# Frankie2030/DataMining_RecBLR

Hardware: AMD Instinct MI355X
Metric: sequences/sec fwd+bwd at B=2048 L=200 d=128; 1/2/4/8-GPU scaling (higher is better)
Workload: dtype f32 I/O, f16x3 split GEMM products

## Files before the change

datamining_recblr_amd/_lib.py:

```python
from __future__ import annotations

import ctypes
import os
import re
import threading

_HERE = os.path.dirname(os.path.abspath(__file__))
LIB_PATH = os.environ.get("RECBLR_LIB") or os.path.join(_HERE, "lib", "libdmrecblr.so")
HEADER_PATH = os.path.join(os.path.dirname(_HERE), "include", "recblr_hip.h")


class RecBLRNativeError(RuntimeError):
    """The HIP extension is missing, failed to load, or a kernel call failed."""


_BY_VALUE = {"int": ctypes.c_int, "int64_t": ctypes.c_int64, "uint64_t": ctypes.c_uint64,
             "float": ctypes.c_float, "double": ctypes.c_double}
_NOT_DECLARATIONS = re.compile(
    r'/\*.*?\*/|//[^\n]*|^[ \t]*#[^\n]*|\btypedef\b(?:[^;{]|\{[^}]*\})*;|extern\s+"C"\s*\{|^\s*\}\s*$',
    re.S | re.M)


def parse_header(text: str) -> dict:
    out = {}
    for decl in _NOT_DECLARATIONS.sub(" ", text).split(";"):
        decl = " ".join(decl.split())
        if not decl:
            continue
        m = re.fullmatch(r"([\w\s*]+?)\s*\b(\w+)\s*\(([^()]*)\)", decl)
        if m is None:
            raise RecBLRNativeError(f"header: not a plain function declaration: {decl!r}")
        ret, name, params = m.groups()
        if re.fullmatch(r"const\s+char\s*\*", ret):
            restype = ctypes.c_char_p
        elif ret in _BY_VALUE:
            restype = _BY_VALUE[ret]
        else:
            raise RecBLRNativeError(f"header: {name}: unsupported return type {ret!r}")
        argtypes = []
        for param in ([] if params.strip() == "void" else params.split(",")):
            words = param.split()
            by_value = " ".join(words[:-1] if len(words) > 1 else words)
            if "*" in param:
                argtypes.append(ctypes.c_void_p)
            elif by_value in _BY_VALUE:
                argtypes.append(_BY_VALUE[by_value])
            else:
                raise RecBLRNativeError(f"header: {name}: unsupported parameter {param.strip()!r}")
        out[name] = (restype, argtypes)
    return out


def _read(path: str) -> str:
    with open(path) as f:
        return f.read()


def _define(text: str, name: str) -> int:
    m = re.search(rf"^[ \t]*#[ \t]*define[ \t]+{name}[ \t]+\(?(-?\d+)\)?[ \t]*$", text, re.M)
    if m is None:
        raise RecBLRNativeError(f"header: no integer #define {name}")
    return int(m.group(1))


_header = _read(HEADER_PATH)
RB_EINVAL = _define(_header, "RB_EINVAL")
RB_TILE = _define(_header, "RB_TILE")
ABI_VERSION = _define(_header, "RB_ABI_VERSION")

SIGNATURES = parse_header(_header)
EXP_SIGNATURES = parse_header(_read(os.path.join(_HERE, "experimental", "recblr_exp.h")))
PROBE_SIGNATURES = parse_header(_read(os.path.join(_HERE, "probes", "recblr_probe.h")))
SESSION_SIGNATURES = parse_header(_read(os.path.join(_HERE, "session", "recblr_session.h")))

_lock = threading.Lock()
_loaded = {}


def _load(path, signatures, missing, version=None, mismatch=None, cache=True,
          hint="") -> ctypes.CDLL:
    with _lock:
        if cache and path in _loaded:
            return _loaded[path]
        if not os.path.exists(path):
            raise RecBLRNativeError(f"{missing}: {path} is missing. Run "
                                    f"`python -m datamining_recblr_amd.build`{hint}.")
        try:
            lib = ctypes.CDLL(path)
        except OSError as exc:
            raise RecBLRNativeError(f"failed to load {path}: {exc}") from exc
        for name, (res, args) in signatures.items():
            fn = getattr(lib, name)
            fn.restype = res
            fn.argtypes = args
        if version is not None and getattr(lib, version)() != ABI_VERSION:
            raise RecBLRNativeError(mismatch.format(getattr(lib, version)(), ABI_VERSION))
        if cache:
            _loaded[path] = lib
        return lib


def load(path: str | None = None) -> ctypes.CDLL:
    return _load(path or LIB_PATH, SIGNATURES, "HIP extension not built", "rb_version",
                 "ABI mismatch: library {} vs binding {}; rebuild", cache=path is None,
                 hint=" (hipcc --offload-arch=gfx950)")


def load_probe() -> ctypes.CDLL:
    return _load(os.path.join(os.path.dirname(LIB_PATH), "libdmrecblr_probe.so"),
                 PROBE_SIGNATURES, "probe library not built")


def load_exp() -> ctypes.CDLL:
    return _load(os.path.join(os.path.dirname(LIB_PATH), "libdmrecblr_exp.so"), EXP_SIGNATURES,
                 "experimental library not built", "rb_exp_version",
                 "experimental library ABI {} vs {}; rebuild")


def load_session() -> ctypes.CDLL:
    return _load(os.path.join(os.path.dirname(LIB_PATH), "libdmrecblr_session.so"),
                 SESSION_SIGNATURES, "session library not built", "rb_session_version",
                 "session library ABI {} vs {}; rebuild")


_fns = {}
_failure_hooks = []


def on_failure(hook) -> None:
    _failure_hooks.append(hook)


def _check(rc: int, name: str, lib: ctypes.CDLL, last_error: str, hooks: bool = True) -> None:
    if rc == 0:
        return
    kind = str(rc)
    if hooks:
        for hook in _failure_hooks:
            hook()
        kind = "invalid argument" if rc == RB_EINVAL else f"hipError {rc}"
    msg = getattr(lib, last_error)()
    raise RecBLRNativeError(f"{name} failed ({kind}): {msg.decode() if msg else ''}")


def call(name: str, *args) -> None:
    fn = _fns.get(name)
    if fn is None:
        fn = _fns[name] = getattr(load(), name)
    rc = fn(*args)
    if rc != 0:
        _check(rc, name, load(), "rb_last_error_string")


def call_probe(name: str, *args) -> None:
    lib = load_probe()
    _check(getattr(lib, name)(*args), name, lib, "rb_probe_last_error_string", hooks=False)
# ... 13 lines not shown
```

datamining_recblr_amd/blocks.py:

```python
from __future__ import annotations

import os

import torch
import torch.nn.functional as F

from . import kernels
from ._lib import RecBLRNativeError
from .linear import (_timed, fire_hooks, has_hooks, linear, mm_nn, mm_nn_dact, mm_nn_dact_ok, mm_nt,
                     mm_nt_act, mm_nt_act_ok, mm_nt_ln, mm_nt_ln_ok, rmax_buffer, wgrad)

__all__ = ["draw_seed", "ResidualGrad", "add_dropout_layer_norm", "embed_dropout_layer_norm",
           "linear_add_dropout_layer_norm", "silu_dropout", "feed_forward", "set_defer_residual",
           "defer_residual"]


_GOLDEN = 0x9E3779B97F4A7C15


def _rank() -> int:
    dist = torch.distributed
    return dist.get_rank() if dist.is_available() and dist.is_initialized() else 0


def draw_seed() -> int:
    s = int(torch.randint(0, 2 ** 62, (1,), dtype=torch.int64).item())
    r = _rank()
    if r:
        s = (s + r * _GOLDEN) % (2 ** 62)
    return s


def _drop(dropout: torch.nn.Dropout, training: bool):
    p = float(dropout.p) if training else 0.0
    return p, (draw_seed() if p > 0.0 else 0)


def _require_gpu(t):
    if t.device.type != "cuda":
        raise RecBLRNativeError(
            "the RecBLR blocks run on the MI355X HIP path only (ROCm GPU tensors)")


class ResidualGrad:
    __slots__ = ("ds", "rows", "taken")

    def __init__(self, rows=None):
        self.ds = None
        self.rows = rows
        self.taken = False


_defer_residual = [os.environ.get("RECBLR_DEFER_RESIDUAL", "1") != "0"]


def set_defer_residual(on: bool) -> None:
    _defer_residual[0] = bool(on)


def defer_residual() -> bool:
    return _defer_residual[0]


# ... 87 lines not shown
        flat = idx.reshape(-1).contiguous()
        plan = None
        if ctx.needs_input_grad[0]:
            plan = kernels.embedding_plan(flat, table.shape[0], table.shape[1])
        y, s, mean, rstd = kernels.add_ln_fwd(table, None, gamma, beta, eps, mask=mask,
                                              seed=seed, p=p, idx=flat, save=save)
        ctx.seed, ctx.p = seed, p
        ctx.padding_idx, ctx.num_rows = padding_idx, table.shape[0]
        ctx.plan = plan
        ctx.addend = _take(addend)
        ctx.save_for_backward(s, mean, rstd, gamma, mask, flat)
        return y.view(*idx.shape, table.shape[1])

    @staticmethod
    def backward(ctx, dy):
        s, mean, rstd, gamma, mask, flat = ctx.saved_tensors
        _, da, dg, db, _ = kernels.add_ln_bwd(dy, s, gamma, mean, rstd, mask=mask,
                                              seed=ctx.seed, p=ctx.p, want_ds=False,
                                              want_da=True, dy2=_pop(ctx.addend))
        dtable = None
        if ctx.needs_input_grad[0]:
            dtable = kernels.embedding_bwd(flat, da, ctx.num_rows, ctx.padding_idx,
                                           plan=ctx.plan)
            ctx.plan = None
        return dtable, None, dg, db, None, None, None, None, None, None


class _SiluDropout(torch.autograd.Function):
    @staticmethod
    def forward(ctx, a, mask, seed, p):
        a = a.contiguous()
        ctx.seed, ctx.p = seed, p
        ctx.save_for_backward(a, mask)
        return kernels.silu_dropout_fwd(a, mask=mask, seed=seed, p=p)

    @staticmethod
    def backward(ctx, du):
        a, mask = ctx.saved_tensors
        da, _ = kernels.silu_dropout_bwd(a, du, mask=mask, seed=ctx.seed, p=ctx.p)
        return da, None, None, None


class _FeedForward(torch.autograd.Function):

    @staticmethod
    def forward(ctx, x, w1, b1, w2, b2, gamma, beta, seed1, seed2, p, eps, in_addend=None,
                out_addend=None, observe=None):
        d = x.shape[-1]
        x2 = x.reshape(-1, d)
        M, inner = x2.shape[0], w1.shape[0]
        f = 2 * M * d * inner
        want = ctx.needs_input_grad[1] or ctx.needs_input_grad[3]
        r_x = rmax_buffer(x2, inner, d) if want else None
        if mm_nt_act_ok(x2, w1):
            (a1, u), a1_bias = _timed("gemm", f, mm_nt_act, x2, w1, b1, seed1, p, rmax=r_x), None
        else:
            a1 = _timed("gemm", f, mm_nt, x2, w1, rmax=r_x)
            u = kernels.silu_dropout_fwd(a1, seed=seed1, p=p, bias=b1)
            a1_bias = b1
        r_u = rmax_buffer(u, d, inner) if want else None
        save = any(ctx.needs_input_grad)
        x2c = x2.contiguous()
        if observe is None and mm_nt_ln_ok(u, w2):
            y, s, mean, rstd = _timed("gemm", f, mm_nt_ln, u, w2, b2, x2c, gamma, beta, eps,
                                      seed2, p, rmax=r_u)
        else:
            a2 = _timed("gemm", f, mm_nt, u, w2, b2, rmax=r_u)
            if observe is not None:
                pre = a1 if a1_bias is None else a1 + a1_bias
                observe(x2.view(x.shape), pre.view(*x.shape[:-1], inner),
                        u.view(*x.shape[:-1], inner), a2.view(x.shape))
            y, s, mean, rstd = kernels.add_ln_fwd(a2, x2c, gamma, beta, eps, seed=seed2, p=p,
                                                  save=save)
        ctx.r_x, ctx.r_u = r_x, r_u
        ctx.seed1, ctx.seed2, ctx.p = seed1, seed2, p
        ctx.a1_has_bias = a1_bias is None
        ctx.in_addend = in_addend if in_addend is not None and in_addend.taken else None
        ctx.out_addend = _take(out_addend)
        ctx.save_for_backward(x2, a1, u, s, mean, rstd, w1, b1, w2, gamma)
        return y.view(x.shape)

    @staticmethod
    def backward(ctx, dy):
        x2, a1, u, s, mean, rstd, w1, b1, w2, gamma = ctx.saved_tensors
        M, d = x2.shape
        f = 2 * M * d * w1.shape[0]
        ds, da2, dgamma, dbeta, db2 = kernels.add_ln_bwd(
            dy, s, gamma, mean, rstd, seed=ctx.seed2, p=ctx.p, want_ds=True, want_da=True,
            want_dbias=True, dy2=_pop(ctx.out_addend))
        r_da2 = rmax_buffer(da2, w2.shape[1], d) if ctx.r_u is not None else None
        if ctx.a1_has_bias and mm_nn_dact_ok(da2, w2):
            da1, db1 = _timed("gemm", f, mm_nn_dact, da2, w2, a1, ctx.seed1, ctx.p, rmax=r_da2)
            dw2 = _timed("gemm", f, wgrad, da2, u, ymax=r_da2, xmax=ctx.r_u)
        else:
            du = _timed("gemm", f, mm_nn, da2, w2, rmax=r_da2)
            dw2 = _timed("gemm", f, wgrad, da2, u, ymax=r_da2, xmax=ctx.r_u)
            da1, db1 = kernels.silu_dropout_bwd(a1, du, seed=ctx.seed1, p=ctx.p, want_dbias=True,
                                                bias=None if ctx.a1_has_bias else b1)
        r_da1 = rmax_buffer(da1, d, w1.shape[0]) if ctx.r_x is not None else None
        dx = _timed("gemm", f, mm_nn, da1, w1, rmax=r_da1)
        if ctx.in_addend is not None:
            ctx.in_addend.ds = ds
        else:
            dx.add_(ds)
        dw1 = _timed("gemm", f, wgrad, da1, x2, ymax=r_da1, xmax=ctx.r_x)
        return (dx.view(dy.shape), dw1, db1, dw2, db2, dgamma, dbeta, None, None, None, None,
                None, None, None)


def add_dropout_layer_norm(a, residual, dropout: torch.nn.Dropout, ln: torch.nn.LayerNorm,
                           training: bool, slot: ResidualGrad | None = None,
                           addend: ResidualGrad | None = None):
    _require_gpu(a)
    if a.shape[-1] not in kernels.ROW_SIZES:
        return ln(dropout(a) + residual)
    p, seed = _drop(dropout, training)
    return _AddDropoutLN.apply(a, residual, ln.weight, ln.bias, None, seed, p, ln.eps, slot,
                               addend)


def linear_add_dropout_layer_norm(x, proj: torch.nn.Linear, residual, dropout: torch.nn.Dropout,
                                  ln: torch.nn.LayerNorm, training: bool,
                                  slot: ResidualGrad | None = None,
                                  addend: ResidualGrad | None = None):
    _require_gpu(x)
    x2 = x.reshape(-1, x.shape[-1])
    if proj.bias is None and ln.weight.shape[0] == proj.weight.shape[0] and mm_nt_ln_ok(x2, proj.weight):
        p, seed = _drop(dropout, training)
        return _LinearAddDropoutLN.apply(x, proj.weight, residual, ln.weight, ln.bias, seed, p,
                                         ln.eps, slot, addend)
    return add_dropout_layer_norm(proj(x), residual, dropout, ln, training, slot, addend)


def embed_dropout_layer_norm(idx, emb: torch.nn.Embedding, dropout: torch.nn.Dropout,
                             ln: torch.nn.LayerNorm, training: bool,
                             addend: ResidualGrad | None = None):
    _require_gpu(emb.weight)
    if emb.weight.shape[1] not in kernels.ROW_SIZES:
        return ln(dropout(emb(idx)))
    p, seed = _drop(dropout, training)
    return _EmbedDropoutLN.apply(emb.weight, idx, ln.weight, ln.bias, None, seed, p, ln.eps,
                                 emb.padding_idx, addend)


def silu_dropout(a, dropout: torch.nn.Dropout, training: bool):
    _require_gpu(a)
    if a.shape[-1] not in kernels.ROW_SIZES:
        return dropout(F.silu(a))
    p, seed = _drop(dropout, training)
    return _SiluDropout.apply(a, None, seed, p)

# ... 20 lines not shown
```

datamining_recblr_amd/build.py:

```python
from __future__ import annotations

import glob
import os
import shutil
import subprocess
import sys

_HERE = os.path.dirname(os.path.abspath(__file__))
ROOT = os.path.dirname(_HERE)
SOURCES = sorted(glob.glob(os.path.join(_HERE, "csrc", "*.hip")))
HEADERS = sorted(glob.glob(os.path.join(_HERE, "csrc", "*.h"))) + [
    os.path.join(ROOT, "include", "recblr_hip.h")]
OUT = os.path.join(_HERE, "lib", "libdmrecblr.so")
PROBE_SOURCES = sorted(glob.glob(os.path.join(_HERE, "probes", "*.hip")))
PROBE_HEADERS = HEADERS + sorted(glob.glob(os.path.join(_HERE, "probes", "*.h")))
PROBE_OUT = os.path.join(_HERE, "lib", "libdmrecblr_probe.so")
EXP_SOURCES = sorted(glob.glob(os.path.join(_HERE, "experimental", "*.hip")))
EXP_HEADERS = HEADERS + sorted(glob.glob(os.path.join(_HERE, "experimental", "*.h")))
EXP_OUT = os.path.join(_HERE, "lib", "libdmrecblr_exp.so")
SESSION_SOURCES = sorted(glob.glob(os.path.join(_HERE, "session", "*.hip")))
SESSION_HEADERS = HEADERS + sorted(glob.glob(os.path.join(_HERE, "session", "*.h")))
SESSION_OUT = os.path.join(_HERE, "lib", "libdmrecblr_session.so")
ARCH = os.environ.get("PYTORCH_ROCM_ARCH", "gfx950")

FLAGS = ["-O3", "-std=c++20", "-shared", "-fPIC", f"--offload-arch={ARCH}",
         "-ffp-contract=off", "-Wall", "-Wno-unused-function"]


def hipcc() -> str:
    for cand in (os.environ.get("HIPCC"), "/opt/rocm/bin/hipcc", shutil.which("hipcc")):
        if cand and os.path.exists(cand):
            return cand
    raise RuntimeError("hipcc not found (expected /opt/rocm/bin/hipcc)")


def _stale(out, deps) -> bool:
    if not os.path.exists(out):
        return True
    t = os.path.getmtime(out)
    return any(os.path.getmtime(s) > t for s in deps)


def _compile(out, sources, extra, verbose, jobs):
    os.makedirs(os.path.dirname(out), exist_ok=True)
    tmp = out + ".tmp"
    cmd = [hipcc(), *FLAGS, *extra, "-I", os.path.join(ROOT, "include"), "-o", tmp, *sources]
    if jobs > 1:
        cmd.insert(1, f"-parallel-jobs={jobs}")
    if verbose:
        print(" ".join(cmd), flush=True)
    subprocess.run(cmd, check=True)
    os.replace(tmp, out)


def build(force: bool = False, verbose: bool = False, jobs: int = 4) -> str:
    if force or _stale(OUT, SOURCES + HEADERS):
        _compile(OUT, SOURCES, [], verbose, jobs)
    if PROBE_SOURCES and (force or _stale(PROBE_OUT, PROBE_SOURCES + PROBE_HEADERS)):
        _compile(PROBE_OUT, PROBE_SOURCES, ["-fvisibility=hidden"], verbose, jobs)
    if EXP_SOURCES and (force or _stale(EXP_OUT, EXP_SOURCES + EXP_HEADERS)):
        _compile(EXP_OUT, EXP_SOURCES, ["-fvisibility=hidden"], verbose, jobs)
    if SESSION_SOURCES and (force or _stale(SESSION_OUT, SESSION_SOURCES + SESSION_HEADERS)):
        _compile(SESSION_OUT, SESSION_SOURCES, ["-fvisibility=hidden"], verbose, jobs)
    return OUT

# ... 4 lines not shown
```

datamining_recblr_amd/csrc/capi.hip:

```cpp
#include "common.h"

#include <atomic>

namespace rb {

namespace {
thread_local std::string g_last_error;
}

int fail(const char* msg) {
  g_last_error = msg;
  return RB_EINVAL;
}

static int fail(const char* fn, const char* msg) {
  g_last_error = std::string(fn) + ": " + msg;
  return RB_EINVAL;
}

int num_cus() {
  static std::atomic<int> cache[64];
  int dev = 0;
  if (hipGetDevice(&dev) != hipSuccess || dev < 0 || dev >= 64) dev = 0;
  int n = cache[dev].load(std::memory_order_relaxed);
// ... 88 lines not shown
  return launch_conv_bwd<T>(x, x_rs, w, bias, g1, g2, dx, dx_rs, dw_part, db_part, B, L, H, K,
                            seq_offsets, as_stream(stream));
}

template <typename T>
int gate_scan_fwd(const char* fn, const T* rg, int64_t rg_rs, const T* xc, int64_t xc_rs,
                  const T* z, int64_t z_rs, const float* lam, const float* gate_b,
                  const float* h0, int64_t h0_bs, T* y, int64_t y_rs, float* carries, int64_t B,
                  int64_t L, int64_t H, const int64_t* seq_offsets, void* stream,
                  T* y_last = nullptr, const int64_t* batch_row = nullptr) {
  if (!rg || !xc || !z || !lam || !(y || y_last)) return fail(fn, "null pointer");
  if (h0_bs != 0 && h0_bs < H) return fail(fn, "h0 batch stride must be 0 or >= H");
  if (rg_rs < 2 * H || xc_rs < H || z_rs < H || y_rs < H) return fail(fn, "row stride too small");
  if (int r = check_dims(B, L, H, max4(rg_rs, xc_rs, z_rs, y_rs))) return r;
  return launch_gate_fwd<T>(rg, rg_rs, xc, xc_rs, z, z_rs, lam, gate_b, h0, h0_bs, y, y_rs,
                            carries, B, L, H, seq_offsets, as_stream(stream), y_last, batch_row);
}

template <typename T>
int gate_scan_bwd(const char* fn, const T* rg, int64_t rg_rs, const T* xc, int64_t xc_rs,
                  const T* z, int64_t z_rs, const float* lam, const float* gate_b,
                  const float* carries, const T* dy, T* drg, int64_t drg_rs, T* dxc,
                  int64_t dxc_rs, T* dz, int64_t dz_rs, float* part, float* dh0_part, int64_t B,
                  int64_t L, int64_t H, const int64_t* seq_offsets, void* stream,
                  const T* dy_last = nullptr, const int64_t* batch_row = nullptr) {
  if (!rg || !xc || !z || !lam || !carries || !(dy || dy_last) || !drg || !dxc || !dz || !part ||
      !dh0_part)
    return fail(fn, "null pointer");
  if (rg_rs < 2 * H || xc_rs < H || z_rs < H || drg_rs < 2 * H || dxc_rs < H || dz_rs < H)
    return fail(fn, "row stride too small");
  if (int r = check_dims(B, L, H, max4(max4(rg_rs, xc_rs, z_rs, drg_rs), dz_rs, dxc_rs, H)))
    return r;
  return launch_gate_bwd<T>(rg, rg_rs, xc, xc_rs, z, z_rs, lam, gate_b, carries, dy, drg, drg_rs,
                            dxc, dxc_rs, dz, dz_rs, part, dh0_part, B, L, H, seq_offsets,
                            as_stream(stream), dy_last, batch_row);
}

const bf16_t* bf(const rb_bf16* p) { return reinterpret_cast<const bf16_t*>(p); }
bf16_t* bf(rb_bf16* p) { return reinterpret_cast<bf16_t*>(p); }

}

DropSpec make_drop(const uint8_t* mask, uint64_t seed, float p) {
  DropSpec d{};
  d.mask = mask;
  d.scale = p > 0.0f ? 1.0f / (1.0f - p) : 1.0f;
  d.key0 = (uint32_t)seed;
  d.key1 = (uint32_t)(seed >> 32);
  const double keep = 1.0 - (double)p;
  d.keep_thresh = keep >= 1.0 ? 0xFFFFFFFFu : (uint32_t)(keep * 4294967296.0);
  d.mode = mask ? 1 : (p > 0.0f ? 2 : 0);
  return d;
}
}

using namespace rb;

extern "C" {

int rb_version(void) { return RB_ABI_VERSION; }

const char* rb_last_error_string(void) { return g_last_error.c_str(); }

int rb_num_kernels(void) { return 24; }

int rb_scan_fwd(const float* gates, const float* tokens, float* states, int64_t B, int64_t C,
                int64_t T, void* stream) {
  return scan_fwd(__func__, gates, tokens, states, B, C, T, stream);
}

int rb_scan_bwd(const float* gates, const float* states, const float* grad, float* d_gates,
                float* d_tokens, int64_t B, int64_t C, int64_t T, void* stream) {
  return scan_bwd(__func__, gates, states, grad, d_gates, d_tokens, B, C, T, stream);
}

int rb_conv_silu_fwd(const float* x, int64_t x_rs, const float* w, const float* bias, float* xc,
                     int64_t xc_rs, int64_t B, int64_t L, int64_t H, int64_t K,
                     const int64_t* seq_offsets, void* stream) {
  return conv_silu_fwd(__func__, x, x_rs, w, bias, xc, xc_rs, B, L, H, K, seq_offsets, stream);
}

int rb_conv_silu_fwd_rows(const float* x, int64_t x_rs, const float* w, const float* bias,
                          float* xc, int64_t xc_rs, int64_t ntok, int64_t H, int64_t K,
                          const int64_t* row_pos, void* stream) {
  return conv_silu_fwd_rows(__func__, x, x_rs, w, bias, xc, xc_rs, ntok, H, K, row_pos, stream);
}

int rb_conv_silu_bwd(const float* x, int64_t x_rs, const float* w, const float* bias,
                     const float* g1, const float* g2, float* dx, int64_t dx_rs, float* dw_part,
                     float* db_part, int64_t B, int64_t L, int64_t H, int64_t K,
                     const int64_t* seq_offsets, void* stream) {
  return conv_silu_bwd(__func__, x, x_rs, w, bias, g1, g2, dx, dx_rs, dw_part, db_part, B, L, H,
                       K, seq_offsets, stream);
}

int rb_gate_scan_fwd(const float* rg, int64_t rg_rs, const float* xc, int64_t xc_rs,
                     const float* z, int64_t z_rs, const float* lam, const float* gate_b,
                     const float* h0, int64_t h0_bs, float* y, int64_t y_rs, float* carries,
                     int64_t B, int64_t L, int64_t H, const int64_t* seq_offsets, void* stream) {
  return gate_scan_fwd(__func__, rg, rg_rs, xc, xc_rs, z, z_rs, lam, gate_b, h0, h0_bs, y, y_rs,
                       carries, B, L, H, seq_offsets, stream);
}

int rb_gate_scan_bwd(const float* rg, int64_t rg_rs, const float* xc, int64_t xc_rs,
                     const float* z, int64_t z_rs, const float* lam, const float* gate_b,
                     const float* carries, const float* dy, float* drg, int64_t drg_rs,
// ... 73 lines not shown
int rb_gate_scan_bwd_bf16(const rb_bf16* rg, int64_t rg_rs, const rb_bf16* xc, int64_t xc_rs,
                          const rb_bf16* z, int64_t z_rs, const float* lam, const float* gate_b,
                          const float* carries, const rb_bf16* dy, rb_bf16* drg, int64_t drg_rs,
                          rb_bf16* dxc, int64_t dxc_rs, rb_bf16* dz, int64_t dz_rs, float* part,
                          float* dh0_part, int64_t B, int64_t L, int64_t H,
                          const int64_t* seq_offsets, void* stream) {
  return gate_scan_bwd(__func__, bf(rg), rg_rs, bf(xc), xc_rs, bf(z), z_rs, lam, gate_b, carries,
                       bf(dy), bf(drg), drg_rs, bf(dxc), dxc_rs, bf(dz), dz_rs, part, dh0_part,
                       B, L, H, seq_offsets, stream);
}

int rb_add_ln_fwd(const float* a, const int64_t* idx, int64_t n_idx_rows, const uint8_t* mask,
                  uint64_t seed, float p, const float* r, const float* gamma, const float* beta,
                  float eps, float* y, float* s_out, float* mean, float* rstd, int64_t rows,
                  int64_t d, void* stream) {
  if (!a || !gamma || !beta || !y) return fail("rb_add_ln_fwd: null pointer");
  if (rows <= 0 || d <= 0) return fail("rb_add_ln_fwd: rows and d must be positive");
  if (idx && n_idx_rows <= 0) return fail("rb_add_ln_fwd: empty gather table");
  if (!(p >= 0.0f && p < 1.0f)) return fail("rb_add_ln_fwd: dropout p must be in [0, 1)");
  if ((s_out == nullptr) != (mean == nullptr) || (mean == nullptr) != (rstd == nullptr))
    return fail("rb_add_ln_fwd: s_out, mean and rstd must be given together");
  return launch_add_ln_fwd(a, idx, n_idx_rows, make_drop(mask, seed, p), r, gamma, beta, eps, y,
                           s_out, mean, rstd, rows, d, reinterpret_cast<hipStream_t>(stream));
}

int64_t rb_row_num_parts(int64_t rows, int64_t width) {
  if (rows <= 0 || width <= 0) return 0;
  return ln_num_parts(rows, width);
}

int rb_add_ln_bwd2(const float* dy, const float* dy2, const float* s, const float* gamma,
                   const float* mean, const float* rstd, const uint8_t* mask, uint64_t seed,
                   float p, float* ds, float* da, float* dgamma_part, float* dbeta_part,
                   float* dbias_part, int64_t n_parts, int64_t rows, int64_t d, void* stream) {
  if (!dy || !s || !gamma || !mean || !rstd || !dgamma_part || !dbeta_part)
    return fail("rb_add_ln_bwd: null pointer");
  if (!ds && !da && !dbias_part) return fail("rb_add_ln_bwd: nothing to write");
  if (rows <= 0 || d <= 0) return fail("rb_add_ln_bwd: rows and d must be positive");
  if (!(p >= 0.0f && p < 1.0f)) return fail("rb_add_ln_bwd: dropout p must be in [0, 1)");
  if (n_parts != ln_num_parts(rows, d)) return fail("rb_add_ln_bwd: n_parts != rb_row_num_parts");
  return launch_add_ln_bwd(dy, dy2, s, gamma, mean, rstd, make_drop(mask, seed, p), ds, da,
                           dgamma_part, dbeta_part, dbias_part, n_parts, rows, d,
                           reinterpret_cast<hipStream_t>(stream));
}

int rb_add_ln_bwd(const float* dy, const float* s, const float* gamma, const float* mean,
                  const float* rstd, const uint8_t* mask, uint64_t seed, float p, float* ds,
                  float* da, float* dgamma_part, float* dbeta_part, float* dbias_part,
                  int64_t n_parts, int64_t rows, int64_t d, void* stream) {
  return rb_add_ln_bwd2(dy, nullptr, s, gamma, mean, rstd, mask, seed, p, ds, da, dgamma_part,
                        dbeta_part, dbias_part, n_parts, rows, d, stream);
}

int rb_silu_dropout_fwd(const float* a, const float* bias, const uint8_t* mask, uint64_t seed,
                        float p, float* u, int64_t rows, int64_t cols, void* stream) {
  if (!a || !u) return fail("rb_silu_dropout_fwd: null pointer");
  if (bias && !aligned16(bias)) return fail("rb_silu_dropout_fwd: misaligned bias");
  if (rows <= 0 || cols <= 0) return fail("rb_silu_dropout_fwd: rows and cols must be positive");
  if (!(p >= 0.0f && p < 1.0f)) return fail("rb_silu_dropout_fwd: dropout p must be in [0, 1)");
  if (!aligned16(a) || !aligned16(u) || (mask && (reinterpret_cast<uintptr_t>(mask) & 3)))
    return fail("rb_silu_dropout_fwd: misaligned buffer");
  return launch_silu_dropout_fwd(a, bias, make_drop(mask, seed, p), u, rows, cols,
                                 reinterpret_cast<hipStream_t>(stream));
}

int rb_silu_dropout_bwd(const float* a, const float* bias, const uint8_t* mask, uint64_t seed,
                        float p, const float* du, float* da, float* dbias_part, int64_t n_parts,
                        int64_t rows, int64_t cols, void* stream) {
  if (!a || !du || !da) return fail("rb_silu_dropout_bwd: null pointer");
  if (bias && !aligned16(bias)) return fail("rb_silu_dropout_bwd: misaligned bias");
  if (rows <= 0 || cols <= 0) return fail("rb_silu_dropout_bwd: rows and cols must be positive");
  if (!(p >= 0.0f && p < 1.0f)) return fail("rb_silu_dropout_bwd: dropout p must be in [0, 1)");
  if (!aligned16(a) || !aligned16(du) || !aligned16(da) ||
      (mask && (reinterpret_cast<uintptr_t>(mask) & 3)))
    return fail("rb_silu_dropout_bwd: misaligned buffer");
  if (dbias_part && n_parts != ln_num_parts(rows, cols))
    return fail("rb_silu_dropout_bwd: n_parts != rb_row_num_parts");
  return launch_silu_dropout_bwd(a, bias, make_drop(mask, seed, p), du, da, dbias_part,
                                 ln_num_parts(rows, cols), rows, cols,
                                 reinterpret_cast<hipStream_t>(stream));
}

int rb_dropout_mask(uint64_t seed, float p, uint8_t* out, int64_t n, void* stream) {
  if (!out) return fail("rb_dropout_mask: null pointer");
  if (n <= 0 || n % 4) return fail("rb_dropout_mask: n must be a positive multiple of 4");
  if (!(p >= 0.0f && p < 1.0f)) return fail("rb_dropout_mask: dropout p must be in [0, 1)");
  return launch_dropout_mask(make_drop(nullptr, seed, p), out, n,
                             reinterpret_cast<hipStream_t>(stream));
}

int64_t rb_embedding_bwd_workspace(int64_t M, int64_t V, int64_t d) {
  if (M <= 0 || V <= 0 || d <= 0) return 0;
  return emb_workspace_bytes(M, V, d);
}

int rb_embedding_bwd_plan(const int64_t* idx, int64_t M, int64_t d, int64_t V, void* workspace,
                          int64_t workspace_bytes, void* stream) {
  if (!idx || !workspace) return fail("rb_embedding_bwd_plan: null pointer");
  if (M <= 0 || d <= 0 || V <= 0) return fail("rb_embedding_bwd_plan: M, d, V must be positive");
  if (M >= (int64_t(1) << 31) || V >= (int64_t(1) << 30))
    return fail("rb_embedding_bwd_plan: M or V too large");
  return launch_embedding_plan(idx, M, d, V, workspace, workspace_bytes,
                               reinterpret_cast<hipStream_t>(stream));
}

int rb_embedding_bwd_apply(const float* grad, int64_t M, int64_t d, int64_t V,
                           int64_t padding_idx, float* dweight, void* workspace,
                           int64_t workspace_bytes, void* stream) {
  if (!grad || !dweight || !workspace) return fail("rb_embedding_bwd_apply: null pointer");
  if (M <= 0 || d <= 0 || V <= 0) return fail("rb_embedding_bwd_apply: M, d, V must be positive");
  if (M >= (int64_t(1) << 31) || V >= (int64_t(1) << 30))
    return fail("rb_embedding_bwd_apply: M or V too large");
  return launch_embedding_apply(grad, M, d, V, padding_idx, dweight, workspace, workspace_bytes,
                                reinterpret_cast<hipStream_t>(stream));
}
// ... 245 lines not shown
int rb_gemm_nt_h_mode(int mode) { return gemm_nt_h_mode(mode); }

int rb_gemm_nt_h_ln(const float* A, int64_t lda, int64_t M, int64_t R, const void* Wf, int64_t C,
                    const float* bias, const float* resid, const float* gamma, const float* beta,
                    float eps, uint64_t seed, float p, float* y, float* s_out, float* mean,
                    float* rstd, int64_t ldo, float* rmax, void* stream) {
  if (!A || !Wf || !resid || !gamma || !beta || !y || !s_out || !mean || !rstd)
    return fail("rb_gemm_nt_h_ln: null pointer");
  if (M <= 0 || R <= 0 || C != 128) return fail("rb_gemm_nt_h_ln: C must be 128, M and R positive");
  if (R != 128 && R != 256 && R != 512) return fail("rb_gemm_nt_h_ln: R must be 128, 256 or 512");
  if (lda < R || lda % 4 || ldo < C || ldo % 4) return fail("rb_gemm_nt_h_ln: bad row strides");
  if (!aligned16(A) || !aligned16(Wf) || !aligned16(resid) || !aligned16(y) || !aligned16(s_out) ||
      !aligned16(gamma) || !aligned16(beta) || (bias && !aligned16(bias)))
    return fail("rb_gemm_nt_h_ln: A, Wf, resid, y, s_out, gamma, beta and bias must be 16-byte aligned");
  if (!(p >= 0.0f && p < 1.0f)) return fail("rb_gemm_nt_h_ln: dropout p must be in [0, 1)");
  if (!(eps > 0.0f)) return fail("rb_gemm_nt_h_ln: eps must be positive");
  if ((M + 31) / 32 > 0x3fffffffLL) return fail("rb_gemm_nt_h_ln: grid too large");
  if (gemm_nt_h_mode(-1) != 1) return fail("rb_gemm_nt_h_ln: needs the weight-stationary kernel (rb_gemm_nt_h_mode 1)");
  return launch_gemm_nt_ws_ln(A, lda, M, (int)R, Wf, (int)C, bias, resid, make_drop(nullptr, seed, p),
                              gamma, beta, eps, y, s_out, mean, rstd, ldo, rmax,
                              reinterpret_cast<hipStream_t>(stream));
}

int rb_gemm_h_split_weights(const rb_split_job* jobs, int64_t n, void* stream) {
  if (!jobs || n < 1 || n > RB_MAX_SPLIT_JOBS)
    return fail("rb_gemm_h_split_weights: need 1..RB_MAX_SPLIT_JOBS jobs");
  for (int64_t j = 0; j < n; ++j) {
    const rb_split_job& b = jobs[j];
    if (!b.W || !b.Wf) return fail("rb_gemm_h_split_weights: null pointer");
    if (b.C <= 0 || b.R <= 0 || b.C % 32 || b.R % 16 || b.C > (1 << 20) || b.R > (1 << 20))
      return fail("rb_gemm_h_split_weights: C must be a multiple of 32 and R of 16");
    if (b.ldw < (b.transpose ? b.C : b.R)) return fail("rb_gemm_h_split_weights: bad row stride");
    if (!aligned16(b.Wf)) return fail("rb_gemm_h_split_weights: Wf must be 16-byte aligned");
  }
  return launch_split_weights_h(jobs, (int)n, reinterpret_cast<hipStream_t>(stream));
}

int rb_gemm_nt_h(const float* A, int64_t lda, int64_t M, int64_t R, const void* Wf, int64_t C,
                 const float* bias, float* out, int64_t ldo, int accumulate, float* rmax,
                 void* stream) {
  if (!A || !Wf || !out) return fail("rb_gemm_nt_h: null pointer");
  if (M <= 0 || R <= 0 || C <= 0) return fail("rb_gemm_nt_h: empty shape");
  if (accumulate) return fail("rb_gemm_nt_h: accumulate is not supported (add the residual in its consumer)");
  if (R % 32 || C % 32 || R > (1 << 16) || C > 1024)
    return fail("rb_gemm_nt_h: R and C must be multiples of 32 (C <= 1024)");
  if (lda < R || lda % 4 || ldo < C || ldo % 2) return fail("rb_gemm_nt_h: bad row strides");
  if (!aligned16(A) || !aligned16(Wf) || (reinterpret_cast<uintptr_t>(out) & 7))
    return fail("rb_gemm_nt_h: A and Wf must be 16-byte aligned, out 8-byte aligned");
  if ((M + 31) / 32 > 0x7fffffffLL) return fail("rb_gemm_nt_h: grid too large");
  return launch_gemm_nt_h(A, lda, M, (int)R, Wf, (int)C, bias, out, ldo, accumulate, rmax,
                          reinterpret_cast<hipStream_t>(stream));
}

int rb_gemm_nt_h_act(const float* A, int64_t lda, int64_t M, int64_t R, const void* Wf, int64_t C,
                     const float* bias, float* out, int64_t ldo, float* rmax, float* act,
                     uint64_t seed, float p, void* stream) {
  if (!A || !Wf || !out || !act) return fail("rb_gemm_nt_h_act: null pointer");
  if (M <= 0 || R <= 0 || C <= 0) return fail("rb_gemm_nt_h_act: empty shape");
  if (R % 32 || C % 32 || R > 1024 || C > 1024)
    return fail("rb_gemm_nt_h_act: R and C must be multiples of 32 (R, C <= 1024)");
  if (lda < R || lda % 4 || ldo < C || ldo % 4) return fail("rb_gemm_nt_h_act: bad row strides");
  if (!aligned16(A) || !aligned16(Wf) || !aligned16(out) || !aligned16(act) ||
      (bias && !aligned16(bias)))
    return fail("rb_gemm_nt_h_act: A, Wf, out, act and bias must be 16-byte aligned");
  if (!(p >= 0.0f && p < 1.0f)) return fail("rb_gemm_nt_h_act: dropout p must be in [0, 1)");
  if ((M + 31) / 32 > 0x7fffffffLL) return fail("rb_gemm_nt_h_act: grid too large");
  return launch_gemm_nt_h_act(A, lda, M, (int)R, Wf, (int)C, bias, out, ldo, rmax, act,
                              make_drop(nullptr, seed, p), reinterpret_cast<hipStream_t>(stream));
}

int rb_adam_step(const rb_adam_job* jobs, int64_t n, double lr, double beta1, double beta2,
                 double eps, double weight_decay, double bc1, double bc2, void* stream) {
  if (!jobs || n <= 0 || n > RB_MAX_ADAM_JOBS) return fail("rb_adam_step: 1..RB_MAX_ADAM_JOBS jobs");
  int64_t blocks = 0;
  for (int64_t j = 0; j < n; ++j) {
    const rb_adam_job& b = jobs[j];
    if (!b.param || !b.grad || !b.exp_avg || !b.exp_avg_sq || b.n <= 0)
      return fail("rb_adam_step: null pointer or empty tensor");
    if (!aligned16(b.param) || !aligned16(b.grad) || !aligned16(b.exp_avg) ||
        !aligned16(b.exp_avg_sq))
      return fail("rb_adam_step: tensors must be 16-byte aligned");
    blocks += (b.n + 1023) / 1024;
  }
  if (blocks > 0x7fffffffLL) return fail("rb_adam_step: too many elements");
  if (!(bc1 > 0.0 && bc2 > 0.0)) return fail("rb_adam_step: bias corrections must be > 0");
  return launch_adam(jobs, (int)n, lr, beta1, beta2, eps, weight_decay, bc1, bc2,
                     reinterpret_cast<hipStream_t>(stream));
}

int64_t rb_gemm_nt_h_dact_parts(void) { return nt_h_dact_parts(); }

int rb_gemm_nt_h_dact(const float* A, int64_t lda, int64_t M, int64_t R, const void* Wf, int64_t C,
                      float* out, int64_t ldo, float* rmax, const float* pre, uint64_t seed,
                      float p, float* dpart, int64_t n_parts, void* stream) {
  if (!A || !Wf || !out || !pre || !dpart) return fail("rb_gemm_nt_h_dact: null pointer");
  if (M <= 0 || R <= 0 || C <= 0) return fail("rb_gemm_nt_h_dact: empty shape");
  if (R % 32 || C % 32 || R > 1024 || C > 512)
    return fail("rb_gemm_nt_h_dact: R and C must be multiples of 32 (R <= 1024, C <= 512)");
  if (lda < R || lda % 4 || ldo < C || ldo % 4) return fail("rb_gemm_nt_h_dact: bad row strides");
  if (!aligned16(A) || !aligned16(Wf) || !aligned16(out) || !aligned16(pre) || !aligned16(dpart))
    return fail("rb_gemm_nt_h_dact: A, Wf, out, pre and dpart must be 16-byte aligned");
  if (!(p >= 0.0f && p < 1.0f)) return fail("rb_gemm_nt_h_dact: dropout p must be in [0, 1)");
  if ((M + 31) / 32 > 0x7fffffffLL) return fail("rb_gemm_nt_h_dact: grid too large");
  return launch_gemm_nt_h_dact(A, lda, M, (int)R, Wf, (int)C, out, ldo, rmax, pre,
                               make_drop(nullptr, seed, p), dpart, n_parts,
                               reinterpret_cast<hipStream_t>(stream));
}

int rb_gemm_tn_h(const float* dY, int64_t ldy, const float* X, int64_t ldx, int64_t M, int64_t N,
                 int64_t K, const float* ymax, const float* xmax, float* parts, int64_t splits,
                 void* stream) {
  if (!dY || !X || !ymax || !xmax || !parts) return fail("rb_gemm_tn_h: null pointer");
  if (M <= 0 || N <= 0 || K <= 0) return fail("rb_gemm_tn_h: empty shape");
  if (N % 128 || K % 128 || N > 65536 || K > 65536)
    return fail("rb_gemm_tn_h: N and K must be multiples of 128 (<= 65536)");
  if (splits < 1 || splits > 65536) return fail("rb_gemm_tn_h: splits must be in [1, 65536]");
  if (ldy < N || ldx < K || ldy % 4 || ldx % 4) return fail("rb_gemm_tn_h: bad row strides");
  if (!aligned16(dY) || !aligned16(X)) return fail("rb_gemm_tn_h: dY and X must be 16-byte aligned");
  if ((N / 128) * (K / 128) * splits > 0x7fffffffLL) return fail("rb_gemm_tn_h: grid too large");
  const int64_t mk = ((M + splits - 1) / splits + 31) / 32 * 32;
  if (mk * (ldy > ldx ? ldy : ldx) * 4 >= 0x7fffffffLL)
    return fail("rb_gemm_tn_h: a row chunk spans 2 GiB or more (use more splits)");
  return launch_gemm_tn_h(dY, ldy, X, ldx, M, (int)N, (int)K, ymax, xmax, parts, (int)splits,
                          reinterpret_cast<hipStream_t>(stream));
}

int rb_gemm_bf16_weight_image(const float* W, int64_t ldw, int64_t C, int64_t R, int transpose,
                              void* img, void* stream) {
  if (!W || !img) return fail("rb_gemm_bf16_weight_image: null pointer");
  if (C <= 0 || R <= 0 || C % 16 || R % 32 || C > 65536 || R > 65536)
    return fail("rb_gemm_bf16_weight_image: C % 16 == 0 and R % 32 == 0 required (<= 65536)");
  if (ldw < (transpose ? C : R)) return fail("rb_gemm_bf16_weight_image: bad row stride");
  if (!aligned16(img)) return fail("rb_gemm_bf16_weight_image: img must be 16-byte aligned");
  return launch_bf16_weight_image(W, ldw, (int)C, (int)R, transpose ? 1 : 0, img,
                                  reinterpret_cast<hipStream_t>(stream));
}

int rb_gemm_nt_bf16(const void* A, int64_t lda, int64_t M, int64_t R, const void* img, int64_t C,
                    const float* bias, void* out, int64_t ldo, void* stream) {
  if (!A || !img || !out) return fail("rb_gemm_nt_bf16: null pointer");
  if (M <= 0 || R <= 0 || C <= 0) return fail("rb_gemm_nt_bf16: empty shape");
  if (R % 64 || C % 256 || R > 16384 || C > 65536)
    return fail("rb_gemm_nt_bf16: R % 64 == 0 (<= 16384) and C % 256 == 0 required");
  if (lda < R || lda % 8 || lda > (1 << 20) || ldo < C || ldo % 8)
    return fail("rb_gemm_nt_bf16: bad row strides (lda % 8 == 0, ldo % 8 == 0)");
  if (!aligned16(A) || !aligned16(img) || !aligned16(out) || (bias && !aligned16(bias)))
    return fail("rb_gemm_nt_bf16: A, img, out and bias must be 16-byte aligned");
  if ((M + 255) / 256 > 0x7fffffffLL / (C / 256) / 2) return fail("rb_gemm_nt_bf16: too many tiles");
  return launch_gemm_nt_bf16(A, lda, M, (int)R, img, (int)C, bias, out, ldo,
                             reinterpret_cast<hipStream_t>(stream));
}

int rb_gemm_tn_hs(const float* dY, int64_t ldy, const float* X, int64_t ldx, int64_t M, int64_t N,
                  int64_t K, float* dw, int accumulate, void* stream) {
  if (!dY || !X || !dw) return fail("rb_gemm_tn_hs: null pointer");
  if (M <= 0 || N <= 0 || K <= 0) return fail("rb_gemm_tn_hs: empty shape");
  if (N % 32 || K % 32 || N > 65536 || K > 65536)
    return fail("rb_gemm_tn_hs: N and K must be multiples of 32");
  if (M > (1 << 24)) return fail("rb_gemm_tn_hs: M too large for the few-rows kernel");
// ... 7 lines not shown
```

datamining_recblr_amd/csrc/common.h:

```cpp
#pragma once

#include <hip/hip_runtime.h>

#include <algorithm>
#include <cstdint>
#include <string>
#include <type_traits>

#include "../../include/recblr_hip.h"

namespace rb {

constexpr int kWave = 64;

int fail(const char* msg);
int launch_status(const char* what);
int num_cus();

inline bool aligned16(const void* p) { return (reinterpret_cast<uintptr_t>(p) & 15) == 0; }

template <class F>
auto dispatch_bool(bool b, F&& f) {
  return b ? f(std::true_type{}) : f(std::false_type{});
}
template <int... Vs, class F>
bool dispatch_int(int v, F&& f) {
  return ((v == Vs ? (f(std::integral_constant<int, Vs>{}), true) : false) || ...);
}

__device__ __forceinline__ float sigm(float x) { return 1.0f / (1.0f + expf(-x)); }
__device__ __forceinline__ float softplus_f(float x) { return x > 20.0f ? x : log1pf(expf(x)); }
__device__ __forceinline__ float dsoftplus_f(float x) { return x > 20.0f ? 1.0f : sigm(x); }
__device__ __forceinline__ float silu_f(float x) { return x / (1.0f + expf(-x)); }
__device__ __forceinline__ float dsilu_f(float x) {
  const float s = sigm(x);
  return s * (1.0f + x * (1.0f - s));
}

constexpr float kLog2e = 1.4426950408889634f;
__device__ __forceinline__ float fexp(float x) { return __builtin_amdgcn_exp2f(x * kLog2e); }
__device__ __forceinline__ float frcp(float x) { return __builtin_amdgcn_rcpf(x); }
__device__ __forceinline__ float fsqrt(float x) { return __builtin_amdgcn_sqrtf(x); }
__device__ __forceinline__ float fsigm(float x) { return frcp(1.0f + fexp(-x)); }
__device__ __forceinline__ float fsilu(float x) { return x * fsigm(x); }
__device__ __forceinline__ float fdsilu(float x) {
  const float s = fsigm(x);
  return s * (1.0f + x * (1.0f - s));
}

typedef float rb_f32x4 __attribute__((ext_vector_type(4)));
typedef float rb_f32x2v __attribute__((ext_vector_type(2)));
typedef uint32_t rb_u32x4 __attribute__((ext_vector_type(4)));
typedef uint32_t rb_u32x2 __attribute__((ext_vector_type(2)));

template <bool NT, typename T>
__device__ __forceinline__ T ld_pol(const T* p) {
  if constexpr (NT) return __builtin_nontemporal_load(p);
  else return *p;
}
template <bool NT, typename T>
__device__ __forceinline__ void st_pol(T v, T* p) {
  if constexpr (NT) __builtin_nontemporal_store(v, p);
  else *p = v;
}
constexpr bool kNT = true;

template <bool NT, int V>
__device__ __forceinline__ void ld_f32(float (&o)[V], const float* p) {
  if constexpr (V == 4) {
    const rb_f32x4 t = ld_pol<NT>(reinterpret_cast<const rb_f32x4*>(p));
    o[0] = t[0]; o[1] = t[1]; o[2] = t[2]; o[3] = t[3];
  } else if constexpr (V == 2) {
    const rb_f32x2v t = ld_pol<NT>(reinterpret_cast<const rb_f32x2v*>(p));
    o[0] = t[0]; o[1] = t[1];
  } else {
#pragma unroll
    for (int v = 0; v < V; ++v) o[v] = ld_pol<NT>(p + v);
  }
}

template <bool NT, int V>
__device__ __forceinline__ void st_f32(float* p, const float (&o)[V]) {
  if constexpr (V == 4) {
    st_pol<NT>(rb_f32x4{o[0], o[1], o[2], o[3]}, reinterpret_cast<rb_f32x4*>(p));
  } else if constexpr (V == 2) {
    st_pol<NT>(rb_f32x2v{o[0], o[1]}, reinterpret_cast<rb_f32x2v*>(p));
  } else {
#pragma unroll
    for (int v = 0; v < V; ++v) st_pol<NT>(o[v], p + v);
  }
}

template <int V>
__device__ __forceinline__ void ldv(float (&o)[V], const float* p) { ld_f32<kNT>(o, p); }
template <int V>
__device__ __forceinline__ void stv(float* p, const float (&o)[V]) { st_f32<kNT>(p, o); }
template <int V>
__device__ __forceinline__ void ldc(float (&o)[V], const float* p) { ld_f32<false>(o, p); }
template <int V>
__device__ __forceinline__ void stc(float* p, const float (&o)[V]) { st_f32<false>(p, o); }
// ... 113 lines not shown
#pragma unroll
    for (int k = 0; k < VH / 2; ++k) unpack2(r.w[h0 / 2 + k], o[2 * k], o[2 * k + 1]);
  }
}
template <int VH, typename T, int V>
__device__ __forceinline__ void pack_part(RawVec<T, V>& r, const float (&o)[VH], int h0) {
  if constexpr (sizeof(T) == 4) {
#pragma unroll
    for (int v = 0; v < VH; ++v) r.w[h0 + v] = o[v];
  } else {
    static_assert(VH % 2 == 0, "packed bf16 pairs");
#pragma unroll
    for (int k = 0; k < VH / 2; ++k) r.w[h0 / 2 + k] = pack2(o[2 * k], o[2 * k + 1]);
  }
}
template <int VH, typename T, int V>
__device__ __forceinline__ void opaque_part(RawVec<T, V>& r, int h0) {
  constexpr int per = sizeof(T) == 2 && V > 1 ? 2 : 1;
#pragma unroll
  for (int k = 0; k < VH / per; ++k) asm volatile("" : "+v"(r.w[h0 / per + k]));
}
template <int V>
__device__ __forceinline__ void stv_raw(float* p, const RawVec<float, V>& r) { st_f32<kNT>(p, r.w); }
template <int V>
__device__ __forceinline__ void stv_raw(bf16_t* p, const RawVec<bf16_t, V>& r) {
  if constexpr (V == 8) {
    st_pol<kNT>(rb_u32x4{r.w[0], r.w[1], r.w[2], r.w[3]}, reinterpret_cast<rb_u32x4*>(p));
  } else if constexpr (V == 4) {
    st_pol<kNT>(rb_u32x2{r.w[0], r.w[1]}, reinterpret_cast<rb_u32x2*>(p));
  } else {
    static_assert(V == 2, "packed bf16 image");
    st_pol<kNT>(r.w[0], reinterpret_cast<uint32_t*>(p));
  }
}

__device__ __forceinline__ uint4 philox4x32_10(uint4 c, uint32_t k0, uint32_t k1) {
#pragma unroll
  for (int i = 0; i < 10; ++i) {
    const uint64_t p0 = (uint64_t)0xD2511F53u * c.x, p1 = (uint64_t)0xCD9E8D57u * c.z;
    const uint32_t lo0 = (uint32_t)p0, hi0 = (uint32_t)(p0 >> 32);
    const uint32_t lo1 = (uint32_t)p1, hi1 = (uint32_t)(p1 >> 32);
    c = make_uint4(hi1 ^ c.y ^ k0, lo1, hi0 ^ c.w ^ k1, lo0);
    k0 += 0x9E3779B9u;
    k1 += 0xBB67AE85u;
  }
  return c;
}

struct DropSpec {
  const uint8_t* mask;
  uint32_t key0, key1, keep_thresh;
  float scale;
  int mode;

  __device__ __forceinline__ void get4(int64_t e, float (&m)[4]) const {
    if (mode == 0) {
      m[0] = m[1] = m[2] = m[3] = 1.0f;
    } else if (mode == 1) {
      const uchar4 t = *reinterpret_cast<const uchar4*>(mask + e);
      m[0] = t.x * scale; m[1] = t.y * scale; m[2] = t.z * scale; m[3] = t.w * scale;
    } else {
      const uint64_t g = (uint64_t)e >> 2;
      const uint4 r = philox4x32_10(make_uint4((uint32_t)g, (uint32_t)(g >> 32), 0u, 0u), key0,
                                    key1);
      m[0] = r.x < keep_thresh ? scale : 0.0f;
      m[1] = r.y < keep_thresh ? scale : 0.0f;
      m[2] = r.z < keep_thresh ? scale : 0.0f;
      m[3] = r.w < keep_thresh ? scale : 0.0f;
    }
  }
};

DropSpec make_drop(const uint8_t* mask, uint64_t seed, float p);


int launch_pack_plan(const int64_t* seq, int64_t seq_rs, const int64_t* offs,
                     const int64_t* order, int64_t B, int64_t* ids, int64_t* pos, int64_t* inv,
                     int64_t* last, hipStream_t st);
template <typename T>
int launch_scan_fwd(const T* gates, const T* tokens, T* states, int64_t rows, int64_t steps,
                    hipStream_t st);
template <typename T>
int launch_scan_bwd(const T* gates, const T* states, const T* grad, T* d_gates, T* d_tokens,
                    int64_t rows, int64_t steps, hipStream_t st);
template <typename T>
int launch_conv_fwd(const T* x, int64_t x_rs, const float* w, const float* bias, T* xc,
                    int64_t xc_rs, int64_t B, int64_t L, int64_t H, int64_t K,
                    const int64_t* offs, hipStream_t st);
template <typename T>
int launch_conv_fwd_rows(const T* x, int64_t x_rs, const float* w, const float* bias, T* xc,
                         int64_t xc_rs, int64_t ntok, int64_t H, int64_t K, const int64_t* pos,
                         hipStream_t st);
template <typename T>
int launch_conv_bwd(const T* x, int64_t x_rs, const float* w, const float* bias, const T* g1,
                    const T* g2, T* dx, int64_t dx_rs, float* dw_part, float* db_part, int64_t B,
                    int64_t L, int64_t H, int64_t K, const int64_t* offs, hipStream_t st);
template <typename T>
int launch_gate_fwd(const T* rg, int64_t rg_rs, const T* xc, int64_t xc_rs, const T* z,
                    int64_t z_rs, const float* lam, const float* gb, const float* h0,
                    int64_t h0_bs, T* y, int64_t y_rs, float* carries, int64_t B, int64_t L,
                    int64_t H, const int64_t* offs, hipStream_t st, T* y_last = nullptr,
                    const int64_t* order = nullptr);
template <typename T>
int launch_gate_bwd(const T* rg, int64_t rg_rs, const T* xc, int64_t xc_rs, const T* z,
                    int64_t z_rs, const float* lam, const float* gb, const float* carries,
                    const T* dy, T* drg, int64_t drg_rs, T* dxc, int64_t dxc_rs, T* dz,
                    int64_t dz_rs, float* part, float* dh0_part, int64_t B, int64_t L, int64_t H,
                    const int64_t* offs, hipStream_t st, const T* dy_last = nullptr,
                    const int64_t* order = nullptr);
int launch_add_ln_fwd(const float* a, const int64_t* idx, int64_t nidx, const DropSpec& drop,
                      const float* r, const float* gamma, const float* beta, float eps, float* y,
                      float* s_out, float* mean, float* rstd, int64_t rows, int64_t d,
                      hipStream_t st);
int launch_add_ln_bwd(const float* dy, const float* dy2, const float* s, const float* gamma,
                      const float* mean, const float* rstd, const DropSpec& drop, float* ds,
                      float* da, float* dgp, float* dbp, float* dbiasp, int64_t nparts,
                      int64_t rows, int64_t d, hipStream_t st);
int64_t ln_num_parts(int64_t rows, int64_t d);
int launch_silu_dropout_fwd(const float* a, const float* bias, const DropSpec& drop, float* u,
                            int64_t rows, int64_t cols, hipStream_t st);
int launch_silu_dropout_bwd(const float* a, const float* bias, const DropSpec& drop,
                            const float* du, float* da, float* dbias_part, int64_t nparts,
                            int64_t rows, int64_t cols, hipStream_t st);
int launch_dropout_mask(const DropSpec& drop, uint8_t* out, int64_t n, hipStream_t st);
int launch_split_weights_h(const rb_split_job* jobs, int n, hipStream_t st);
int launch_bf16_weight_image(const float* W, int64_t ldw, int C, int R, int transpose, void* img,
                             hipStream_t st);
int launch_gemm_nt_bf16(const void* A, int64_t lda, int64_t M, int R, const void* img, int C,
                        const float* bias, void* out, int64_t ldo, hipStream_t st);
int launch_gemm_tn_h(const float* Y, int64_t ldy, const float* X, int64_t ldx, int64_t M, int N,
                     int K, const float* ymax, const float* xmax, float* parts, int S,
                     hipStream_t st);
constexpr int kWeightScale = 14;
template <class S>
struct WeightSlot {
  S slot;
  int col, k0;
};
template <class S = int64_t, class I>
__host__ __device__ inline WeightSlot<S> weight_slot32(int nkb, I cb, int kb, int p, int lane) {
  return {((S)(cb * nkb + kb) * 2 + p) * 64 + lane, (int)cb * 32 + (lane & 31),
          kb * 16 + 8 * (lane >> 5)};
}
template <class S = int64_t, class I>
__host__ __device__ inline WeightSlot<S> weight_slot16(int nkb, I cb, int ks, int p, int lane) {
  return {((S)(cb * nkb + ks) * 2 + p) * 64 + lane, (int)cb * 16 + (lane & 15),
          ks * 32 + 8 * (lane >> 4)};
}
__host__ __device__ inline int64_t ws_image_offset(int64_t C, int64_t K) {
  return C * K * 4 + ((C * 4 + 15) / 16) * 16;
}
struct WeightImage {
  const void* wf;
  const int* ew;
  const void* wi;
};
inline WeightImage weight_image(const void* Wf, int64_t C, int64_t R) {
  const char* base = static_cast<const char*>(Wf);
  return {Wf, reinterpret_cast<const int*>(base + C * R * 4), base + ws_image_offset(C, R)};
}
int nt_dact_zero_rest(float* dpart, int64_t used, int64_t n_parts, int C, hipStream_t st);
bool nt_ws_ok(int64_t M, int K, int C, const float* A, int64_t lda, const float* out, int64_t ldo);
int launch_gemm_nt_ws(const float* A, int64_t lda, int64_t M, int K, const void* Wf, int C,
                      const float* bias, float* out, int64_t ldo, float* rmax, hipStream_t st);
int gemm_nt_h_mode(int mode);
bool nt_ws_act_ok(int64_t M, int K, int C, const float* A, int64_t lda, const float* out,
                  const float* other, int64_t ldo);
int launch_gemm_nt_ws_act(const float* A, int64_t lda, int64_t M, int K, const void* Wf, int C,
                          const float* bias, float* out, int64_t ldo, float* rmax, float* act,
                          DropSpec drop, hipStream_t st);
int launch_gemm_nt_ws_dact(const float* A, int64_t lda, int64_t M, int K, const void* Wf, int C,
                           float* out, int64_t ldo, float* rmax, const float* pre, DropSpec drop,
                           float* dpart, int64_t n_parts, hipStream_t st);
// ... 76 lines not shown
```

datamining_recblr_amd/csrc/gemm_half.hip:

```cpp
#include "common.h"
#include "f16x3.h"
#include "nt_plan.h"

#include <type_traits>

namespace rb {
namespace {

constexpr int kTA = 4;
constexpr int kHead = 11;
constexpr int kTRedo = 14;
constexpr int kSent = -4096;

struct SplitJobsH {
  const float* W[RB_MAX_SPLIT_JOBS];
  f16x8* Wf[RB_MAX_SPLIT_JOBS];
  int64_t ldw[RB_MAX_SPLIT_JOBS];
  int C[RB_MAX_SPLIT_JOBS], R[RB_MAX_SPLIT_JOBS], tr[RB_MAX_SPLIT_JOBS];
  int bstart[RB_MAX_SPLIT_JOBS + 1];
  int n;
};

__global__ void __launch_bounds__(256) k_split_weights_h(const SplitJobsH jobs) {
  __shared__ float smax[256];
// ... 217 lines not shown
  f32x16 acc[N_NB];
#pragma unroll
  for (int n = 0; n < N_NB; ++n)
#pragma unroll
    for (int e = 0; e < 16; ++e) acc[n][e] = 0.0f;

  a_tile();
  b_tile();
  issueB();
  for (int a = 0; a < N_LA && a < U; ++a) issueA();

  const uint32_t smem_base = (uint32_t)(uintptr_t)(lds_ptr_t)smem;
  const uint32_t s_ew_addr = smem_base + N_RING;
  const uint32_t s_bias_addr = smem_base + N_RING + N_MAXC * 4;
  uint32_t a_rd[2][2];
  {
    const int row = wave * 32 + (lane & 31);
    const int sw = (row >> 1) & 7;
#pragma unroll
    for (int s = 0; s < 2; ++s)
#pragma unroll
      for (int c = 0; c < 2; ++c)
        a_rd[s][c] = row * 128 + (((4 * s + 2 * (lane >> 5) + c) ^ sw) << 4);
  }
  const int ccol = lane & 31;
  auto crow = [&](int j) { return 8 * (j >> 2) + 4 * (lane >> 5) + (j & 3); };

  int er = kSent;
  float scl = 1.0f, thr = 0.0f;
  float tmax = 0.0f;
  bool flag_tile = false;
  int nflag = 0;
  int* s_flag = reinterpret_cast<int*>(smem + N_RING + N_MAXC * 8) + wave * N_MAXFLAG;

  f32x16 pend[DEFER ? N_NB : 1];
  float pbias[N_NB];
  int pend_q = N_NB;
  bool pend_on = false, pend_full = true;
  const char* pend_base = nullptr;
  int64_t pend_r0 = 0;
  int pend_c0 = 0;
  const int st_lane = WIDE ? (int)(((4 * (lane >> 5) + (lane & 3)) * ldo + (lane & 28)) * 4)
                           : (int)((4 * (lane >> 5)) * ldo * 4) + ccol * 4;
  auto store_block = [&](const f32x16& blk, int n) {
    if constexpr (WIDE) {
#pragma unroll
      for (int g = 0; g < 4; ++g) {
        float v[4];
#pragma unroll
        for (int r = 0; r < 4; ++r) v[r] = BIAS ? blk[4 * g + r] + pbias[n] : blk[4 * g + r];
        quad_transpose(v, lane);
        f32x4* o = (f32x4*)(pend_base + (int64_t)(8 * g) * ldo * 4 + n * 128 + st_lane);
        const int64_t row = pend_r0 + 8 * g + 4 * (lane >> 5) + (lane & 3);
        if (pend_full || row < M)
          __builtin_nontemporal_store(f32x4{v[0], v[1], v[2], v[3]}, o);
        if constexpr (ACT) {
          float m[4];
          drop.get4(e_base + row * C + pend_c0 + n * 32 + (lane & 28), m);
          f32x4 a;
#pragma unroll
          for (int r = 0; r < 4; ++r) a[r] = fsilu(v[r]) * m[r];
          if (pend_full || row < M)
            __builtin_nontemporal_store(a, (f32x4*)(reinterpret_cast<char*>(o) + act_delta));
        }
      }
    } else {
#pragma unroll
      for (int j = 0; j < 16; ++j) {
        const int rj = 8 * (j >> 2) + (j & 3);
        float* o = (float*)(pend_base + (int64_t)rj * ldo * 4 + n * 128 + st_lane);
        const float v = BIAS ? blk[j] + pbias[n] : blk[j];
        if (pend_full || pend_r0 + crow(j) < M) __builtin_nontemporal_store(v, o);
      }
    }
  };
  const int rq = 4 * (lane >> 5) + (lane & 3);
  auto ld_pre = [&](int n, f32x4 (&q)[4]) {
    if constexpr (DACT) {
#pragma unroll
      for (int g = 0; g < 4; ++g) {
        const int64_t row = pend_r0 + 8 * g + rq;
        int64_t off = (int64_t)(8 * g) * ldo * 4 + n * 128 + st_lane + pre_delta;
        if (!pend_full && row >= M) off -= (row - (M - 1)) * ldo * 4;
        q[g] = *reinterpret_cast<const f32x4*>(pend_base + off);
      }
    }
  };
  auto dact_block = [&](const f32x16& blk, int n, const f32x4 (&pq)[4], bool skip_sums) {
    if constexpr (DACT) {
      float cs[4] = {0.0f, 0.0f, 0.0f, 0.0f};
#pragma unroll
      for (int g = 0; g < 4; ++g) {
        float v[4];
#pragma unroll
        for (int r = 0; r < 4; ++r) v[r] = blk[4 * g + r];
        quad_transpose(v, lane);
        const int64_t row = pend_r0 + 8 * g + rq;
        const bool ok = pend_full || row < M;
        float mk[4];
        drop.get4(e_base + row * C + pend_c0 + n * 32 + (lane & 28), mk);
        const f32x4 pv = pq[g];
        f32x4 d;
#pragma unroll
        for (int r = 0; r < 4; ++r) d[r] = (v[r] * mk[r]) * fdsilu(pv[r] + 0.0f);
        if (ok) {
          __builtin_nontemporal_store(
              d, (f32x4*)(pend_base + (int64_t)(8 * g) * ldo * 4 + n * 128 + st_lane));
#pragma unroll
          for (int r = 0; r < 4; ++r) cs[r] += d[r];
        }
      }
      if (!skip_sums) {
#pragma unroll
        for (int r = 0; r < 4; ++r) {
          cs[r] += dpp_xor1(cs[r]);
          cs[r] += dpp_xor2(cs[r]);
          cs[r] += __shfl_xor(cs[r], 32);
        }
        if ((lane & 3) == 0 && lane < 32) {
#pragma unroll
          for (int r = 0; r < 4; ++r) s_col[pend_c0 + n * 32 + (lane & 28) + r] += cs[r];
        }
      }
    }
  };
  f32x4 pq1[4];
  bool pend_skip = false;
  auto store_quarter = [&]() {
    const int q = pend_q++;
    if constexpr (DEFER && DACT) {
      if (q == 0) dact_block(pend[0], 0, pq1, pend_skip);
      else if (q == 1) dact_block(pend[1], 1, pq1, pend_skip);
      else if (q == 2) dact_block(pend[2], 2, pq1, pend_skip);
      else dact_block(pend[3], 3, pq1, pend_skip);
      if (q + 1 < N_NB) ld_pre(q + 1, pq1);
    } else if constexpr (DEFER) {
      if (q == 0) store_block(pend[0], 0);
      else if (q == 1) store_block(pend[1], 1);
      else if (q == 2) store_block(pend[2], 2);
      else store_block(pend[3], 3);
    }
    return pend_full;
  };
  auto dact_epilogue = [&](bool skip_sums) {
    if constexpr (DACT && !DEFER) {
      f32x4 pq[2][4];
      ld_pre(0, pq[0]);
#pragma unroll
      for (int n = 0; n < N_NB; ++n) {
        if (n + 1 < N_NB) ld_pre(n + 1, pq[(n + 1) & 1]);
        dact_block(acc[n], n, pq[n & 1], skip_sums);
      }
    }
  };
  bool stored_prev = false;

  int i = 0, kt = 0, c_slot_a = 0, c_slot_b = 0;
// ... 160 lines not shown
      ++kt;
    }
  }
  while (pend_on && pend_q < N_NB) store_quarter();

  if (nflag > 0) {
    wait_vm<0>();
    const int ntodo = nflag > N_MAXFLAG ? my_tiles : nflag;
    if (DACT && nflag > N_MAXFLAG)
      for (int c = lane; c < C; c += 64) s_col[c] = 0.0f;
    for (int f = 0; f < ntodo; ++f) {
      const int ii = nflag > N_MAXFLAG ? f : s_flag[f];
      int mt, ct;
      tile_of(ii, mt, ct);
      if (mt >= m_tiles) continue;
      int64_t row = (int64_t)mt * N_BM + wave * 32 + (lane & 31);
      if (row >= M) row = M - 1;
      const float* arow = A + row * lda + 8 * (lane >> 5);
      float m = 0.0f;
      for (int kb = 0; kb < KB16; ++kb) {
        const f32x4 p = *reinterpret_cast<const f32x4*>(arow + kb * 16);
        const f32x4 q = *reinterpret_cast<const f32x4*>(arow + kb * 16 + 4);
        m = fmaxf(m, max8abs(p, q));
      }
      m = fmaxf(m, __shfl_xor(m, 32));
      const int e = exp_of(m);
      const float sc = __builtin_amdgcn_ldexpf(1.0f, kTRedo - e);
      int erow[16];
#pragma unroll
      for (int j = 0; j < 16; ++j) erow[j] = __shfl(e, crow(j)) - kTRedo - kWeightScale;
      for (int n = 0; n < N_NB; ++n) {
        f32x16 c;
#pragma unroll
        for (int j = 0; j < 16; ++j) c[j] = 0.0f;
        for (int kb = 0; kb < KB16; ++kb) {
          const f32x4 p = *reinterpret_cast<const f32x4*>(arow + kb * 16);
          const f32x4 q = *reinterpret_cast<const f32x4*>(arow + kb * 16 + 4);
          f16x8 a0, a1;
          split8(p, q, sc, a0, a1);
          const f16x8* bp = Wf + ((int64_t)((ct * N_NB + n) * KB16 + kb) * 2) * 64 + lane;
          const f16x8 b0 = bp[0], b1 = bp[64];
          c = mfma3_h(a0, a1, b0, b1, c);
        }
        const int col = ct * N_BN + n * 32 + ccol;
        const int ecol = s_ew[col];
        const float bv = BIAS ? s_bias[col] : 0.0f;
        float csum = 0.0f;
#pragma unroll
        for (int j = 0; j < 16; ++j) {
          const int64_t r = (int64_t)mt * N_BM + wave * 32 + crow(j);
          if (r < M) {
            float v = __builtin_amdgcn_ldexpf(c[j], erow[j] + ecol) + bv;
            if constexpr (DACT) {
              float mk[4];
              const int64_t ei = e_base + r * C + col;
              drop.get4(ei & ~(int64_t)3, mk);
              const int q = (int)(ei & 3);
              v = (v * (q == 0 ? mk[0] : q == 1 ? mk[1] : q == 2 ? mk[2] : mk[3])) *
                  fdsilu(pre[r * ldo + col] + 0.0f);
              csum += v;
            }
            out[r * ldo + col] = v;
            if constexpr (ACT) {
              float mk[4];
              const int64_t ei = e_base + r * C + col;
              drop.get4(ei & ~(int64_t)3, mk);
              const int q = (int)(ei & 3);
              act[r * ldo + col] = fsilu(v) * (q == 0 ? mk[0] : q == 1 ? mk[1] : q == 2 ? mk[2] : mk[3]);
            }
          }
        }
        if constexpr (DACT) {
          csum += __shfl_xor(csum, 32);
          if (lane < 32) s_col[col] += csum;
        }
      }
    }
  }
  if constexpr (DACT) {
    __syncthreads();
    const float* s_all = reinterpret_cast<const float*>(smem + CF::LDS);
    for (int c = tid; c < C; c += N_THREADS) {
      float t = s_all[c];
#pragma unroll
      for (int w = 1; w < N_WAVES; ++w) t += s_all[w * N_DACT_MAXC + c];
      dpart[(int64_t)bid * C + c] = t;
    }
  }
}

template <bool BIAS, bool WIDE, int NB, bool ACT = false, bool DACT = false>
__global__ void __launch_bounds__(N_THREADS, 1) k_gemm_nt_h(const float* __restrict__ A, int64_t lda,
                                                          int64_t M, int R,
                                                          const f16x8* __restrict__ Wf,
                                                          const int* __restrict__ ew, int C,
                                                          const float* __restrict__ bias,
                                                          float* __restrict__ out, int64_t ldo,
                                                          float* __restrict__ rmax, int m_tiles,
                                                          float* __restrict__ act, DropSpec drop,
                                                          int64_t e_base,
                                                          const float* __restrict__ pre,
                                                          float* __restrict__ dpart) {
  extern __shared__ __attribute__((aligned(16))) char smem[];
  nt_h_body<BIAS, WIDE, NB, ACT, DACT>(smem, (int)blockIdx.x, (int)gridDim.x, A, lda, M, R, Wf, ew,
                                       C, bias, out, ldo, rmax, m_tiles, act, drop, e_base, pre,
                                       dpart);
}

struct NtPhase {
  const float* A;
  int64_t M;
  float* out;
  float* rmax;
  float* act;
  const float* pre;
  float* dpart;
  int64_t e_base;
  int m_tiles;
  int grid;
};

template <bool BIAS, int NB, bool ACT = false, bool DACT = false>
// ... 532 lines not shown
```

datamining_recblr_amd/csrc/gemm_ws.hip:

```cpp
#include "common.h"
#include "f16x3.h"

#include <type_traits>
#include <utility>

namespace rb {
namespace ws {

constexpr int kTR = 14;
constexpr int WAVES = 8, THREADS = 64 * WAVES, RB = 32;

template <int K, int NCB_, int D_>
struct Cfg {
  static constexpr int KS = K / 32;
  static constexpr int NCB = NCB_;
  static constexpr int D = D_;
  static constexpr int WC = 16 * NCB;
  static constexpr int NT = WC * WAVES;
  static constexpr int NLD = K / 64;
  static constexpr int IMG = RB * K * 4;
  static constexpr int NST = 2 * NCB;
  static constexpr int INFO = 2 * IMG;
  static constexpr int COLS = INFO + 2 * RB * 8;
  static constexpr int STATS = COLS + NT * 8;
  static constexpr bool STG = K <= 256;
  static constexpr int STAGE = STATS + 2 * 2 * RB * WAVES * 4;
  static constexpr int LDS = STAGE + (STG ? D * WAVES * NLD * 1024 : 0);
  static_assert(KS * NCB <= 16 && NCB >= 1, "B slice <= 128 VGPRs");
  static_assert(LDS <= 160 * 1024, "LDS");
};

__device__ __forceinline__ f32x4 gload16(const char* base, uint32_t off) {
  return *reinterpret_cast<const f32x4*>(base + off);
}
__device__ __forceinline__ void dma16(__amdgpu_buffer_rsrc_t rs, uint32_t lds, uint32_t voff) {
  __builtin_amdgcn_raw_ptr_buffer_load_lds(rs, (__attribute__((address_space(3))) void*)(uintptr_t)lds, 16,
                                           voff, 0, 0, 0);
}

struct LnSpec {
  const float* gamma = nullptr;
  const float* beta = nullptr;
  float eps = 0.0f;
  float* mean = nullptr;
  float* rstd = nullptr;
};

template <int K, int NCB, int D, bool BIAS, bool DEFER, int ABL, int EPI = 0>
__global__ void __launch_bounds__(THREADS, 1)
k_gemm_nt_ws(const float* __restrict__ A, int64_t lda, int64_t M, const f16x8* __restrict__ Wi,
             const int* __restrict__ ew, int C, const float* __restrict__ bias,
             float* __restrict__ out, int64_t ldo, float* __restrict__ rmax,
             float* __restrict__ act, DropSpec drop, const float* __restrict__ pre,
             float* __restrict__ dpart, LnSpec ln) {
  using CF = Cfg<K, NCB, D>;
  constexpr int KS = CF::KS, WC = CF::WC, NT = CF::NT, NLD = CF::NLD, NST = CF::NST;
  constexpr bool TWO = EPI == 1 || EPI == 3;
  constexpr bool PRE = EPI == 2 || EPI == 3;
  constexpr int NSTT = TWO ? 2 * NST : NST;
  constexpr int NPRE = PRE ? 2 * NCB : 0;
  constexpr int NSO = NSTT + 1 + (EPI == 3 ? 2 : 0);
  static_assert(EPI != 3 || (NCB == 1 && DEFER), "LN epilogue: whole 128-column rows, deferred stores");
  constexpr bool EARLY1 = D == 1 && (ABL & 32) == 0;
  extern __shared__ __attribute__((aligned(16))) char smem[];
  const int tid = threadIdx.x, lane = tid & 63;
  const int wave = __builtin_amdgcn_readfirstlane(tid >> 6);
  const int bid = blockIdx.x, G = gridDim.x;
  const int nct = C / NT;
  const int ct = (bid >> 3) % nct;
  const int64_t nrb = (M + RB - 1) / RB;
  const int64_t rb0 = (int64_t)(bid / (8 * nct)) * 8 + (bid & 7);
  const int64_t rbs = (int64_t)(G / (8 * nct)) * 8;
  const int nb = rb0 < nrb ? (int)((nrb - 1 - rb0) / rbs + 1) : 0;
  const int64_t prow = (int64_t)(bid / (8 * nct)) * 8 + (bid & 7);
  if (nb == 0) {
    if constexpr (EPI == 2)
      for (int c = tid; c < NT; c += THREADS) dpart[prow * C + ct * NT + c] = 0.0f;
    return;
  }

  const uint32_t sbase = (uint32_t)(uintptr_t)(__attribute__((address_space(3))) void*)smem;
  const uint32_t s_info = sbase + CF::INFO;
  const uint32_t s_cols = sbase + CF::COLS;
  for (int c = tid; c < NT; c += THREADS) {
    const int e = ew[ct * NT + c] - kTR - kWeightScale;
    const float bv = BIAS ? bias[ct * NT + c] : 0.0f;
    asm volatile("ds_write_b32 %0, %1" ::"v"(s_cols + c * 4), "v"(e) : "memory");
    asm volatile("ds_write_b32 %0, %1" ::"v"(s_cols + (NT + c) * 4), "v"(bv) : "memory");
  }

  const int col0 = ct * NT + wave * WC;
  f16x8 bw[NCB][KS][2];
#pragma unroll
  for (int cb = 0; cb < NCB; ++cb)
#pragma unroll
    for (int s = 0; s < KS; ++s)
#pragma unroll
      for (int p = 0; p < 2; ++p)
        bw[cb][s][p] = Wi[weight_slot16(KS, col0 / 16 + cb, s, p, lane).slot];

  const int my_row = 4 * wave + (lane >> 4);
  uint32_t woff[NLD];
#pragma unroll
  for (int j = 0; j < NLD; ++j) {
    const int c = 16 * j + (lane & 15);
    const int r16 = my_row & 15, rb16 = my_row >> 4;
    const int s = c >> 3, g = (c >> 1) & 3, half = c & 1;
    const int pos = (r16 ^ ((4 * s + g) & 15)) + 16 * g;
    woff[j] = (uint32_t)(((rb16 * KS + s) * 2) * 1024 + pos * 16 + half * 8);
  }
  f32x4 ra[CF::STG ? 1 : D][NLD];
  auto blk_r0 = [&](int b) __attribute__((always_inline)) -> int64_t { return (rb0 + (int64_t)b * rbs) * RB; };
  auto rsrc_of = [&](const float* p, int64_t r0, int64_t ld) __attribute__((always_inline)) {
    const uint64_t u = reinterpret_cast<uint64_t>(p + r0 * ld);
    const uint64_t ub = (uint64_t)(uint32_t)__builtin_amdgcn_readfirstlane((uint32_t)u) |
                        ((uint64_t)(uint32_t)__builtin_amdgcn_readfirstlane((uint32_t)(u >> 32)) << 32);
    const int64_t n = M - r0 < RB ? (M - r0 > 0 ? M - r0 : 0) : RB;
    return __builtin_amdgcn_make_buffer_rsrc(reinterpret_cast<void*>(ub), 0, (int)(n * ld * 4), 0x00020000);
  };
  const uint32_t a_voff = (uint32_t)(my_row * lda * 4) + (uint32_t)(lane & 15) * 16;
  const uint32_t s_stage = sbase + CF::STAGE;
  auto stage_of = [&](int set) __attribute__((always_inline)) -> uint32_t { return s_stage + (uint32_t)((set * WAVES + wave) * NLD) * 1024; };
  auto issue = [&](int b, f32x4 (&dst)[NLD], int set) __attribute__((always_inline)) {
    if constexpr ((ABL & 8) != 0) return;
    const auto rs = rsrc_of(A, blk_r0(b), lda);
    if constexpr (CF::STG) {
      const uint32_t st = __builtin_amdgcn_readfirstlane(stage_of(set));
#pragma unroll
      for (int j = 0; j < NLD; ++j)
// ... 65 lines not shown
    rd(std::integral_constant<int, 0>{}, 0);
    auto unit = [&](auto uc) __attribute__((always_inline)) {
      constexpr int u = decltype(uc)::value, t = u & 1, s = u >> 1, r = u & 1;
      if constexpr ((ABL & 16) != 0) {
        asm volatile("s_waitcnt lgkmcnt(0)" : "+v"(fa[0][0]), "+v"(fa[0][1]));
        fa[1][0] = fa[0][0]; fa[1][1] = fa[0][1];
      } else if constexpr (u + 1 < 2 * KS) {
        rd(std::integral_constant<int, u + 1>{}, t ^ 1);
        asm volatile("s_waitcnt lgkmcnt(2)" : "+v"(fa[t][0]), "+v"(fa[t][1]));
      } else {
        asm volatile("s_waitcnt lgkmcnt(0)" : "+v"(fa[t][0]), "+v"(fa[t][1]));
      }
#pragma unroll
      for (int cb = 0; cb < NCB; ++cb) {
        acc[r][cb] = mfma3_16(bw[cb][s][0], bw[cb][s][1], fa[t][0], fa[t][1], acc[r][cb]);
      }
      hook(uc);
    };
    [&]<int... U>(std::integer_sequence<int, U...>) __attribute__((always_inline)) {
      (unit(std::integral_constant<int, U>{}), ...);
    }(std::make_integer_sequence<int, 2 * KS>{});
  };

  const uint32_t ldo4 = (uint32_t)ldo * 4;
  f32x4 pend[NST];
  uint32_t soff[NST];
#pragma unroll
  for (int r = 0; r < 2; ++r) {
    if constexpr (NCB == 1) {
      soff[r] = (uint32_t)((16 * r + (lane & 15)) * ldo4) + (uint32_t)(col0 + 4 * (lane >> 4)) * 4;
    } else {
#pragma unroll
      for (int q = 0; q < NCB / 2; ++q) {
        const uint32_t off = (uint32_t)((16 * r + (lane & 7)) * ldo4) +
                             (uint32_t)(col0 + 32 * q + 16 * ((lane >> 3) & 1) + 4 * (lane >> 4)) * 4;
        soff[(q * 2 + r) * 2] = off;
        soff[(q * 2 + r) * 2 + 1] = off + 8 * ldo4;
      }
    }
  }
  __amdgpu_buffer_rsrc_t pending_rs = rsrc_of(out, M, ldo);
  f32x4 pend2[TWO ? NST : 1];
  __amdgpu_buffer_rsrc_t pending_act = rsrc_of(TWO ? act : out, M, ldo);
  auto flush = [&](int i) __attribute__((always_inline)) {
    if constexpr ((ABL & 4) == 0) {
      if (i < NST)
        __builtin_amdgcn_raw_buffer_store_b128(__builtin_bit_cast(u32x4, pend[i]), pending_rs, soff[i], 0, 2);
      else if constexpr (TWO)
        __builtin_amdgcn_raw_buffer_store_b128(__builtin_bit_cast(u32x4, pend2[i - NST]), pending_act,
                                               soff[i - NST], 0, 2);
    }
  };
  f32x4 prv[PRE ? 2 : 1][PRE ? NCB : 1];
  f32x4 csum[EPI == 2 ? NCB : 1];
  if constexpr (EPI == 2)
#pragma unroll
    for (int cb = 0; cb < NCB; ++cb) csum[cb] = f32x4{0.0f, 0.0f, 0.0f, 0.0f};
  auto load_pre = [&](int b) __attribute__((always_inline)) {
    if constexpr (PRE) {
      const auto rs = rsrc_of(pre, blk_r0(b), ldo);
#pragma unroll
      for (int r = 0; r < 2; ++r)
#pragma unroll
        for (int cb = 0; cb < NCB; ++cb)
          prv[r][cb] = __builtin_bit_cast(f32x4, __builtin_amdgcn_raw_buffer_load_b128(
              rs, (uint32_t)((16 * r + (lane & 15)) * ldo4) + (uint32_t)(col0 + 16 * cb + 4 * (lane >> 4)) * 4,
              0, 0));
      asm volatile("" ::: "memory");
    }
  };
  const uint32_t s_stats = sbase + CF::STATS;
  constexpr uint32_t kQ = 2 * RB * WAVES * 4;
  f32x4 gm{}, bt{};
  float lmu[2] = {0.0f, 0.0f}, lrs[2] = {0.0f, 0.0f};
  if constexpr (EPI == 3) {
    gm = *reinterpret_cast<const f32x4*>(ln.gamma + col0 + 4 * (lane >> 4));
    bt = *reinterpret_cast<const f32x4*>(ln.beta + col0 + 4 * (lane >> 4));
  }
  auto ln_part = [&](f32x4 sv, int ib, int r) __attribute__((always_inline)) {
    float m = ((sv[0] + sv[1]) + (sv[2] + sv[3])) * 0.25f;
    float q = 0.0f;
#pragma unroll
    for (int i = 0; i < 4; ++i) {
      const float d = sv[i] - m;
      q += d * d;
    }
#pragma unroll
    for (int o = 16, n2 = 2; o <= 32; o <<= 1, n2 <<= 1) {
      const float mo = __shfl_xor(m, o), qo = __shfl_xor(q, o);
      const float d = mo - m;
      m = (m + mo) * 0.5f;
      q = (q + qo) + (d * d) * (float)n2;
    }
    if (lane < 16) {
      const uint32_t a = s_stats + ((ib * RB + 16 * r + lane) * WAVES + wave) * 4;
      asm volatile("ds_write_b32 %0, %1" ::"v"(a), "v"(m) : "memory");
      asm volatile("ds_write_b32 %0, %1 offset:%2" ::"v"(a), "v"(q), "n"(kQ) : "memory");
    }
  };
  auto normalize = [&](int ibp) __attribute__((always_inline)) {
    f32x4 pm[2][2], pq[2][2];
#pragma unroll
    for (int r = 0; r < 2; ++r) {
      const uint32_t a = s_stats + ((ibp * RB + 16 * r + (lane & 15)) * WAVES) * 4;
      pm[r][0] = lds_read16<f32x4>(a);
      pm[r][1] = lds_read16o<16, f32x4>(a);
      pq[r][0] = lds_read16o<kQ, f32x4>(a);
      pq[r][1] = lds_read16o<kQ + 16, f32x4>(a);
// ... 19 lines not shown
      lrs[r] = rs;
    }
  };
  auto ln_store = [&](int bprev) __attribute__((always_inline)) {
    const int64_t r0 = bprev >= 0 ? blk_r0(bprev) : M;
    const bool mine = wave == 0 && r0 < M;
    const int64_t n = mine ? (M - r0 < RB ? M - r0 : RB) : 0;
    const uint32_t off = lane < RB ? (uint32_t)lane * 4 : 0x40000000u;
    const float* bases[2] = {ln.mean, ln.rstd};
    const float vals[2] = {lane < 16 ? lmu[0] : lmu[1], lane < 16 ? lrs[0] : lrs[1]};
#pragma unroll
    for (int k = 0; k < 2; ++k) {
      const uint64_t u = reinterpret_cast<uint64_t>(bases[k] + (mine ? r0 : 0));
      const uint64_t ub = (uint64_t)(uint32_t)__builtin_amdgcn_readfirstlane((uint32_t)u) |
                          ((uint64_t)(uint32_t)__builtin_amdgcn_readfirstlane((uint32_t)(u >> 32)) << 32);
      const auto rr = __builtin_amdgcn_make_buffer_rsrc(reinterpret_cast<void*>(ub), 0, (int)(n * 4), 0x00020000);
      __builtin_amdgcn_raw_buffer_store_b32(__float_as_uint(vals[k]), rr, off, 0, 0);
    }
  };
  auto finish = [&](int b, int ib) __attribute__((always_inline)) {
    const int64_t r0 = blk_r0(b);
    int er[2];
    er[0] = lds_read_i32(s_info + (ib * RB + (lane & 15)) * 4);
    er[1] = lds_read_i32(s_info + (ib * RB + 16 + (lane & 15)) * 4);
    constexpr int NG = NCB == 1 ? 1 : 2;
#pragma unroll
    for (int q = 0; q < NCB / NG; ++q) {
      i32x4 ec[NG];
      f32x4 bc[NG];
#pragma unroll
      for (int g = 0; g < NG; ++g) {
        const int cb = NG * q + g;
        ec[g] = lds_read16<i32x4>(s_cols + (wave * WC + cb * 16 + 4 * (lane >> 4)) * 4);
        if (BIAS) bc[g] = lds_read16<f32x4>(s_cols + (NT + wave * WC + cb * 16 + 4 * (lane >> 4)) * 4);
        else bc[g] = f32x4{0.0f, 0.0f, 0.0f, 0.0f};
      }
      if constexpr (NG == 1)
        asm volatile("s_waitcnt lgkmcnt(0)" : "+v"(er[0]), "+v"(er[1]), "+v"(ec[0]), "+v"(bc[0]));
      else
        asm volatile("s_waitcnt lgkmcnt(0)" : "+v"(er[0]), "+v"(er[1]), "+v"(ec[0]), "+v"(bc[0]),
                     "+v"(ec[1]), "+v"(bc[1]));
#pragma unroll
      for (int r = 0; r < 2; ++r) {
        f32x4 v[NG];
        f32x4 av[NG];
        const int64_t row = r0 + 16 * r + (lane & 15);
#pragma unroll
        for (int g = 0; g < NG; ++g) {
#pragma unroll
          for (int i = 0; i < 4; ++i) {
            v[g][i] = __builtin_amdgcn_ldexpf(acc[r][NG * q + g][i], er[r] + ec[g][i]);
            if (BIAS) v[g][i] += bc[g][i];
          }
          if constexpr (EPI != 0) {
            float mk[4];
            drop.get4(row * C + col0 + 16 * (NG * q + g) + 4 * (lane >> 4), mk);
            if constexpr (EPI == 1) {
#pragma unroll
              for (int i = 0; i < 4; ++i) av[g][i] = fsilu(v[g][i]) * mk[i];
            } else if constexpr (EPI == 2) {
              const f32x4 pv = prv[r][NG * q + g];
#pragma unroll
              for (int i = 0; i < 4; ++i) v[g][i] = (v[g][i] * mk[i]) * fdsilu(pv[i] + 0.0f);
              csum[NG * q + g] += v[g];
            } else {
              const f32x4 pv = prv[r][NG * q + g];
#pragma unroll
              for (int i = 0; i < 4; ++i) v[g][i] = v[g][i] * mk[i] + pv[i];
            }
          }
        }
        if constexpr (NG == 1) {
          pend[r] = v[0];
          if constexpr (EPI == 1) pend2[r] = av[0];
          if constexpr (EPI == 3) ln_part(v[0], ib, r);
        } else {
          f32x4 x1, x2;
#pragma unroll
          for (int i = 0; i < 4; ++i) {
            const float f0 = v[0][i], f1 = v[1][i];
            const int a0 = __float_as_int(f0), a1 = __float_as_int(f1);
            x1[i] = __int_as_float(__builtin_amdgcn_update_dpp(a0, a1, 0x128, 0xF, 0xC, false));
            x2[i] = __int_as_float(__builtin_amdgcn_update_dpp(a1, a0, 0x128, 0xF, 0x3, false));
          }
          pend[(q * 2 + r) * 2] = x1;
          pend[(q * 2 + r) * 2 + 1] = x2;
          if constexpr (EPI == 1) {
#pragma unroll
            for (int i = 0; i < 4; ++i) {
              const float f0 = av[0][i], f1 = av[1][i];
              const int a0 = __float_as_int(f0), a1 = __float_as_int(f1);
              x1[i] = __int_as_float(__builtin_amdgcn_update_dpp(a0, a1, 0x128, 0xF, 0xC, false));
              x2[i] = __int_as_float(__builtin_amdgcn_update_dpp(a1, a0, 0x128, 0xF, 0x3, false));
            }
            pend2[(q * 2 + r) * 2] = x1;
            pend2[(q * 2 + r) * 2 + 1] = x2;
          }
        }
      }
    }
    pending_rs = rsrc_of(out, r0, ldo);
    if constexpr (TWO) pending_act = rsrc_of(act, r0, ldo);
  };
  auto rmax_store = [&](int b, int ib) __attribute__((always_inline)) {
    const int64_t r0 = blk_r0(b);
    float x = 0.0f;
    if (lane < RB)
      asm volatile("ds_read_b32 %0, %1\n\ts_waitcnt lgkmcnt(0)" : "=v"(x) : "v"(s_info + (2 * RB + ib * RB + lane) * 4));
#pragma unroll
    for (int o = 32; o >= 1; o >>= 1) x = fmaxf(x, __shfl_xor(x, o));
    const bool mine = rmax != nullptr && ct == 0 && wave == 0 && r0 < M;
    const uint64_t u = reinterpret_cast<uint64_t>(rmax) + (mine ? (uint64_t)(r0 / RB) * 4 : 0);
    const uint64_t ub = (uint64_t)(uint32_t)__builtin_amdgcn_readfirstlane((uint32_t)u) |
                        ((uint64_t)(uint32_t)__builtin_amdgcn_readfirstlane((uint32_t)(u >> 32)) << 32);
    const auto rr = __builtin_amdgcn_make_buffer_rsrc(reinterpret_cast<void*>(ub), 0, mine ? 4 : 0, 0x00020000);
    __builtin_amdgcn_raw_buffer_store_b32(__float_as_uint(x), rr, 0, 0, 0);
  };

  [&]<int... P>(std::integer_sequence<int, P...>) __attribute__((always_inline)) {
    (issue(P, ra[CF::STG ? 0 : P], P), ...);
  }(std::make_integer_sequence<int, D>{});
  if constexpr (CF::STG) wait_vm<(D - 1) * NLD>();
  split(ra[0], 0, 0);
  if constexpr (EARLY1) {
    if (wave >= 4) issue(1, ra[0], 0);
  }
  asm volatile("s_waitcnt lgkmcnt(0)" ::: "memory");
  __builtin_amdgcn_s_barrier();

  auto loop = [&](auto late_c) __attribute__((always_inline)) {
    constexpr bool LATE = decltype(late_c)::value;
    constexpr int YS = (LATE ? D : D - 1) * NSO + D * NPRE + (D - 1) * NLD;
    constexpr int Y0 = (D - 1) * NLD + NPRE + (LATE ? NSO : 0);
    auto body = [&](int b, auto par) __attribute__((always_inline)) {
      constexpr int P = decltype(par)::value;
      const int ib = b & 1;
      auto do_split = [&]() __attribute__((always_inline)) {
        if constexpr (CF::STG) {
          if (b >= D - 1) wait_vm<(YS > 63 ? 63 : YS)>();
          else wait_vm<(Y0 > 63 ? 63 : Y0)>();
        }
        split(ra[CF::STG ? 0 : (P + 1) % D], ib ^ 1, (P + 1) % D);
      };
      if constexpr (EARLY1 && !LATE) {
        do_split();
        issue(b + 2, ra[0], 0);
        load_pre(b);
      } else {
        issue(b + D, ra[CF::STG ? 0 : P], P);
        load_pre(b);
        if constexpr (!LATE) do_split();
      }
      if constexpr (DEFER) {
        constexpr int U = 2 * KS, STEP = U / NSTT;
        static_assert(STEP >= 1, "more stores than MFMA units");
        if constexpr (EPI == 3) normalize(ib ^ 1);
        multiply(ib, [&](auto uc) __attribute__((always_inline)) {
          constexpr int u = decltype(uc)::value;
          if constexpr (u % STEP == 0 && u / STEP < NSTT) flush(u / STEP);
        });
        rmax_store(b, ib);
        if constexpr (EPI == 3) ln_store(b - 1);
        finish(b, ib);
      } else {
        multiply(ib, [](auto) __attribute__((always_inline)) {});
        finish(b, ib);
#pragma unroll
        for (int i = 0; i < NSTT; ++i) flush(i);
        rmax_store(b, ib);
      }
      if constexpr (LATE) do_split();
      asm volatile("s_waitcnt lgkmcnt(0)" ::: "memory");
      __builtin_amdgcn_s_barrier();
    };
    for (int b = 0; b < nb; b += D) {
      [&]<int... P>(std::integer_sequence<int, P...>) __attribute__((always_inline)) {
        (body(b + P, std::integral_constant<int, P>{}), ...);
      }(std::make_integer_sequence<int, D>{});
    }
  };
  if ((D == 1 && !EARLY1) || wave < 4) loop(std::true_type{});
  else loop(std::false_type{});
  if constexpr (DEFER) {
    const int blast = (nb + D - 1) / D * D - 1;
    if constexpr (EPI == 3) normalize(blast & 1);
#pragma unroll
    for (int i = 0; i < NSTT; ++i) flush(i);
    if constexpr (EPI == 3) ln_store(blast);
  }
  if constexpr (EPI == 2) {
#pragma unroll
    for (int cb = 0; cb < NCB; ++cb) {
#pragma unroll
      for (int i = 0; i < 4; ++i) {
        float x = csum[cb][i];
        x += dpp_xor1(x);
        x += dpp_xor2(x);
        x += __builtin_bit_cast(float, __builtin_amdgcn_mov_dpp(__builtin_bit_cast(int, x), 0x124, 0xF, 0xF, false));
        x += __builtin_bit_cast(float, __builtin_amdgcn_mov_dpp(__builtin_bit_cast(int, x), 0x128, 0xF, 0xF, false));
        csum[cb][i] = x;
      }
      if ((lane & 15) == 0)
        *reinterpret_cast<f32x4*>(dpart + prow * C + col0 + 16 * cb + 4 * (lane >> 4)) = csum[cb];
    }
  }
}

template <int K, int NCB, int D, bool BIAS, bool DEFER, int ABL, int EPI = 0>
void run(const float* A, int64_t lda, int64_t M, const void* Wi, const int* ew, int C,
         const float* bias, float* out, int64_t ldo, float* rmax, int grid, hipStream_t st,
         float* act = nullptr, DropSpec drop = DropSpec{}, const float* pre = nullptr,
         float* dpart = nullptr, LnSpec ln = LnSpec{}) {
  using CF = Cfg<K, NCB, D>;
  static bool done = false;
  if (!done) {
    (void)hipFuncSetAttribute((const void*)k_gemm_nt_ws<K, NCB, D, BIAS, DEFER, ABL, EPI>,
                              hipFuncAttributeMaxDynamicSharedMemorySize, CF::LDS);
    done = true;
  }
  k_gemm_nt_ws<K, NCB, D, BIAS, DEFER, ABL, EPI><<<grid, THREADS, CF::LDS, st>>>(
      A, lda, M, (const f16x8*)Wi, ew, C, bias, out, ldo, rmax, act, drop, pre, dpart, ln);
}

template <int K>
constexpr int depth() { return K == 512 ? 1 : K == 256 ? 2 : 3; }

inline int ncb_for(int K, int C) {
  int ncb = 16 / (K / 32);
  while (ncb > 1 && C % (128 * ncb)) ncb >>= 1;
  return C % (128 * ncb) ? 0 : ncb;
}

inline int grid_for(int64_t M, int C, int ncb) {
  const int nct = C / (128 * ncb);
  const int unit = 8 * nct;
  int grid = num_cus() / unit * unit;
  const int64_t items = (M + RB - 1) / RB * nct;
  if (items < grid) grid = (int)((items + unit - 1) / unit * unit);
  return grid;
}

}

bool nt_ws_ok(int64_t M, int K, int C, const float* A, int64_t lda, const float* out, int64_t ldo) {
  return (K == 128 || K == 256 || K == 512) && ws::ncb_for(K, C) > 0 && aligned16(A) &&
         lda % 4 == 0 && aligned16(out) && ldo % 4 == 0 && M > 0 &&
         (M + ws::RB - 1) / ws::RB <= 0x3fffffffLL;
}

int launch_gemm_nt_ws(const float* A, int64_t lda, int64_t M, int K, const void* Wf, int C,
                      const float* bias, float* out, int64_t ldo, float* rmax, hipStream_t st) {
  if (!nt_ws_ok(M, K, C, A, lda, out, ldo)) return fail("rb_gemm_nt_h: no weight-stationary launch for this shape");
  const WeightImage w = weight_image(Wf, C, K);
  const int ncb = ws::ncb_for(K, C);
  const int grid = ws::grid_for(M, C, ncb);
  dispatch_int<128, 256, 512>(K, [&](auto kc) {
    dispatch_int<1, 2, 4>(ncb, [&](auto nc) {
      dispatch_bool(bias != nullptr, [&](auto bias_c) {
        constexpr int KK = decltype(kc)::value, NC = decltype(nc)::value;
        if constexpr (NC <= 16 / (KK / 32))
          ws::run<KK, NC, ws::depth<KK>(), decltype(bias_c)::value, true, 0>(
              A, lda, M, w.wi, w.ew, C, bias, out, ldo, rmax, grid, st);
      });
    });
  });
  return launch_status("rb_gemm_nt_h");
}

bool nt_ws_act_ok(int64_t M, int K, int C, const float* A, int64_t lda, const float* out,
                  const float* other, int64_t ldo) {
  return K == 128 && C % 256 == 0 && nt_ws_ok(M, K, C, A, lda, out, ldo) && aligned16(other);
}

int launch_gemm_nt_ws_act(const float* A, int64_t lda, int64_t M, int K, const void* Wf, int C,
                          const float* bias, float* out, int64_t ldo, float* rmax, float* act,
                          DropSpec drop, hipStream_t st) {
  if (!nt_ws_act_ok(M, K, C, A, lda, out, act, ldo)) return fail("rb_gemm_nt_h_act: shape");
  const WeightImage w = weight_image(Wf, C, K);
  const int grid = ws::grid_for(M, C, 2);
  dispatch_bool(bias != nullptr, [&](auto bias_c) {
    ws::run<128, 2, ws::depth<128>(), decltype(bias_c)::value, true, 0, 1>(
        A, lda, M, w.wi, w.ew, C, bias, out, ldo, rmax, grid, st, act, drop);
  });
  return launch_status("rb_gemm_nt_h_act");
}

int launch_gemm_nt_ws_dact(const float* A, int64_t lda, int64_t M, int K, const void* Wf, int C,
                           float* out, int64_t ldo, float* rmax, const float* pre, DropSpec drop,
                           float* dpart, int64_t n_parts, hipStream_t st) {
  if (!nt_ws_act_ok(M, K, C, A, lda, out, pre, ldo)) return fail("rb_gemm_nt_h_dact: shape");
  const WeightImage w = weight_image(Wf, C, K);
  const int grid = ws::grid_for(M, C, 2);
  const int64_t used = grid / (C / 256);
  if (used > n_parts) return fail("rb_gemm_nt_h_dact: dpart has too few rows");
  ws::run<128, 2, ws::depth<128>(), false, true, 0, 2>(A, lda, M, w.wi, w.ew, C, nullptr, out, ldo, rmax, grid,
                                                      st, nullptr, drop, pre, dpart);
  const int rc = launch_status("rb_gemm_nt_h_dact");
  return rc ? rc : nt_dact_zero_rest(dpart, used, n_parts, C, st);
}

bool nt_ws_ln_ok(int64_t M, int K, int C, const float* A, int64_t lda, const float* y,
                 const float* s_out, const float* resid, int64_t ldo) {
  return C == 128 && nt_ws_ok(M, K, C, A, lda, y, ldo) && ws::ncb_for(K, C) == 1 &&
         aligned16(s_out) && aligned16(resid);
}

int launch_gemm_nt_ws_ln(const float* A, int64_t lda, int64_t M, int K, const void* Wf, int C,
                         const float* bias, const float* resid, DropSpec drop, const float* gamma,
                         const float* beta, float eps, float* y, float* s_out, float* mean,
                         float* rstd, int64_t ldo, float* rmax, hipStream_t st) {
  if (!nt_ws_ln_ok(M, K, C, A, lda, y, s_out, resid, ldo) || !gamma || !beta || !mean || !rstd ||
      !aligned16(gamma) || !aligned16(beta))
    return fail("rb_gemm_nt_h_ln: shape, alignment or null pointer");
  const WeightImage w = weight_image(Wf, C, K);
  const int grid = ws::grid_for(M, C, 1);
  ws::LnSpec ln;
  ln.gamma = gamma;
  ln.beta = beta;
  ln.eps = eps;
  ln.mean = mean;
  ln.rstd = rstd;
  dispatch_int<128, 256, 512>(K, [&](auto kc) {
    dispatch_bool(bias != nullptr, [&](auto bias_c) {
      constexpr int KK = decltype(kc)::value;
      ws::run<KK, 1, ws::depth<KK>(), decltype(bias_c)::value, true, 0, 3>(
          A, lda, M, w.wi, w.ew, C, bias, s_out, ldo, rmax, grid, st, y, drop, resid, nullptr, ln);
    });
  });
  return launch_status("rb_gemm_nt_h_ln");
}

}
```

datamining_recblr_amd/csrc/rownorm.hip:

```cpp
#include "common.h"

namespace rb {
namespace {

constexpr bool kLnFwdNT = true, kLnBwdNT = true;
template <bool NT, int V>
__device__ __forceinline__ void st_ln(float* p, const float (&o)[V]) {
  if constexpr (NT) stv(p, o); else stc(p, o);
}

template <int LPR>
__device__ __forceinline__ float row_sum(float v) {
#pragma unroll
  for (int o = LPR / 2; o > 0; o >>= 1) v += __shfl_xor(v, o, kWave);
  return v;
}

constexpr int kRowBlocks = 1024;
constexpr int kRowBlocksFwd = 4 * kRowBlocks;

template <int NV, int LPR>
__global__ void __launch_bounds__(256)
k_add_ln_fwd(const float* __restrict__ a, const int64_t* __restrict__ idx, int64_t nidx,
             DropSpec drop, const float* __restrict__ r, const float* __restrict__ gamma,
// ... 125 lines not shown
#pragma unroll
    for (int k = 0; k < NV; ++k) {
      const int c = (l + k * LPR) * 4;
      float d[4];
#pragma unroll
      for (int v = 0; v < 4; ++v) d[v] = ok ? rs * (g[k][v] - mg - xh[k][v] * mgx) : 0.0f;
      if (ok && ds_out) st_ln<kLnBwdNT>(ds_out + row * D + c, d);
      if (da_out || dbias_part) {
        float m[4];
        drop.get4(rr * D + c, m);
#pragma unroll
        for (int v = 0; v < 4; ++v) {
          d[v] = d[v] * m[v];
          acca[k][v] += d[v];
        }
        if (ok && da_out) st_ln<kLnBwdNT>(da_out + row * D + c, d);
      }
    }
  }
#pragma unroll
  for (int k = 0; k < NV; ++k)
#pragma unroll
    for (int v = 0; v < 4; ++v)
#pragma unroll
      for (int o = LPR; o < kWave; o <<= 1) {
        accg[k][v] += __shfl_xor(accg[k][v], o, kWave);
        accb[k][v] += __shfl_xor(accb[k][v], o, kWave);
        acca[k][v] += __shfl_xor(acca[k][v], o, kWave);
      }
  if (sub == 0) {
#pragma unroll
    for (int k = 0; k < NV; ++k) {
      const int c = (l + k * LPR) * 4;
#pragma unroll
      for (int v = 0; v < 4; ++v) {
        red[0][wv][c + v] = accg[k][v];
        red[1][wv][c + v] = accb[k][v];
        red[2][wv][c + v] = acca[k][v];
      }
    }
  }
  __syncthreads();
  for (int c = threadIdx.x; c < D; c += blockDim.x) {
    const int64_t o = (int64_t)blockIdx.x * D + c;
    dgamma_part[o] = ((red[0][0][c] + red[0][1][c]) + red[0][2][c]) + red[0][3][c];
    dbeta_part[o] = ((red[1][0][c] + red[1][1][c]) + red[1][2][c]) + red[1][3][c];
    if (dbias_part) dbias_part[o] = ((red[2][0][c] + red[2][1][c]) + red[2][2][c]) + red[2][3][c];
  }
}

template <int NV, int LPR>
__global__ void __launch_bounds__(256)
k_silu_dropout_fwd(const float* __restrict__ a, const float* __restrict__ bias, DropSpec drop,
                   float* __restrict__ u, int64_t rows) {
  constexpr int C = LPR * NV * 4;
  constexpr int RPW = kWave / LPR;
  const int lane = threadIdx.x & (kWave - 1);
  const int sub = lane / LPR;
  const int l = lane - sub * LPR;
  float bv[NV][4];
#pragma unroll
  for (int k = 0; k < NV; ++k) {
    if (bias) {
      ldc(bv[k], bias + (l + k * LPR) * 4);
    } else {
#pragma unroll
      for (int v = 0; v < 4; ++v) bv[k][v] = 0.0f;
    }
  }
  const int64_t wave = (int64_t)blockIdx.x * 4 + (threadIdx.x >> 6);
  const int64_t nwaves = (int64_t)gridDim.x * 4;
  for (int64_t row0 = wave * RPW; row0 < rows; row0 += nwaves * RPW) {
    const int64_t row = row0 + sub;
    if (row >= rows) continue;
#pragma unroll
    for (int k = 0; k < NV; ++k) {
      const int64_t e = row * C + (l + k * LPR) * 4;
      float x[4], m[4], o[4];
      ldv(x, a + e);
      drop.get4(e, m);
#pragma unroll
      for (int v = 0; v < 4; ++v) o[v] = fsilu(x[v] + bv[k][v]) * m[v];
      stv(u + e, o);
    }
  }
}

template <int NV, int LPR>
__global__ void __launch_bounds__(256)
k_silu_dropout_bwd(const float* __restrict__ a, const float* __restrict__ bias, DropSpec drop,
                   const float* __restrict__ du, float* __restrict__ da,
                   float* __restrict__ dbias_part, int64_t rows) {
  constexpr int C = LPR * NV * 4;
  constexpr int RPW = kWave / LPR;
  __shared__ float red[4][C];
  const int lane = threadIdx.x & (kWave - 1);
  const int wv = threadIdx.x >> 6;
  const int sub = lane / LPR;
  const int l = lane - sub * LPR;
  float bv[NV][4];
#pragma unroll
  for (int k = 0; k < NV; ++k) {
    if (bias) {
      ldc(bv[k], bias + (l + k * LPR) * 4);
    } else {
#pragma unroll
      for (int v = 0; v < 4; ++v) bv[k][v] = 0.0f;
    }
  }
  const int64_t wave = (int64_t)blockIdx.x * 4 + wv;
  const int64_t nwaves = (int64_t)gridDim.x * 4;
  float acc[NV][4];
#pragma unroll
  for (int k = 0; k < NV; ++k)
#pragma unroll
    for (int v = 0; v < 4; ++v) acc[k][v] = 0.0f;
  for (int64_t row0 = wave * RPW; row0 < rows; row0 += nwaves * RPW) {
    const int64_t row = row0 + sub;
    if (row >= rows) continue;
#pragma unroll
    for (int k = 0; k < NV; ++k) {
      const int64_t e = row * C + (l + k * LPR) * 4;
      float x[4], g[4], m[4], o[4];
      ldv(x, a + e);
      ldv(g, du + e);
      drop.get4(e, m);
#pragma unroll
      for (int v = 0; v < 4; ++v) {
        o[v] = (g[v] * m[v]) * fdsilu(x[v] + bv[k][v]);
        acc[k][v] += o[v];
      }
      stv(da + e, o);
    }
  }
  if (dbias_part == nullptr) return;
#pragma unroll
  for (int k = 0; k < NV; ++k)
#pragma unroll
    for (int v = 0; v < 4; ++v)
#pragma unroll
      for (int o = LPR; o < kWave; o <<= 1) acc[k][v] += __shfl_xor(acc[k][v], o, kWave);
  if (sub == 0) {
#pragma unroll
    for (int k = 0; k < NV; ++k)
#pragma unroll
      for (int v = 0; v < 4; ++v) red[wv][(l + k * LPR) * 4 + v] = acc[k][v];
  }
  __syncthreads();
  for (int c = threadIdx.x; c < C; c += blockDim.x)
    dbias_part[(int64_t)blockIdx.x * C + c] = ((red[0][c] + red[1][c]) + red[2][c]) + red[3][c];
}

__global__ void k_dropout_mask(DropSpec drop, uint8_t* __restrict__ out, int64_t n4) {
  for (int64_t i = (int64_t)blockIdx.x * blockDim.x + threadIdx.x; i < n4;
       i += (int64_t)gridDim.x * blockDim.x) {
    float m[4];
    drop.get4(i * 4, m);
    uchar4 o;
    o.x = m[0] != 0.0f; o.y = m[1] != 0.0f; o.z = m[2] != 0.0f; o.w = m[3] != 0.0f;
    reinterpret_cast<uchar4*>(out)[i] = o;
  }
}

template <int LPR, int MAXB = kRowBlocks>
int64_t row_blocks(int64_t rows) {
  constexpr int RPB = 4 * (kWave / LPR);
  return std::max<int64_t>(1, std::min<int64_t>(MAXB, (rows + RPB - 1) / RPB));
}

template <int NV, int LPR>
int add_ln_fwd_t(const float* a, const int64_t* idx, int64_t nidx, const DropSpec& drop,
                 const float* r, const float* gamma, const float* beta, float eps, float* y,
                 float* s_out, float* mean, float* rstd, int64_t rows, hipStream_t st) {
  hipLaunchKernelGGL((k_add_ln_fwd<NV, LPR>), dim3((unsigned)row_blocks<LPR, kRowBlocksFwd>(rows)),
                     dim3(256), 0,
                     st, a, idx, nidx, drop, r, gamma, beta, eps, y, s_out, mean, rstd, rows);
  return launch_status("rb_add_ln_fwd");
}

template <int NV, int LPR>
int add_ln_bwd_t(const float* dy, const float* dy2, const float* s, const float* gamma,
                 const float* mean, const float* rstd, const DropSpec& drop, float* ds, float* da,
                 float* dgp, float* dbp, float* dbiasp, int64_t nparts, int64_t rows,
                 hipStream_t st) {
  hipLaunchKernelGGL((k_add_ln_bwd<NV, LPR>), dim3((unsigned)nparts), dim3(256), 0, st, dy, dy2, s,
                     gamma, mean, rstd, drop, ds, da, dgp, dbp, dbiasp, rows);
  return launch_status("rb_add_ln_bwd");
}

template <int NV, int LPR>
int silu_fwd_t(const float* a, const float* bias, const DropSpec& drop, float* u, int64_t rows,
               hipStream_t st) {
  hipLaunchKernelGGL((k_silu_dropout_fwd<NV, LPR>),
                     dim3((unsigned)(row_blocks<LPR, 2 * kRowBlocksFwd>(rows))),
                     dim3(256), 0, st, a, bias, drop, u, rows);
  return launch_status("rb_silu_dropout_fwd");
}

template <int NV, int LPR>
int silu_bwd_t(const float* a, const float* bias, const DropSpec& drop, const float* du, float* da,
               float* dbias_part, int64_t nparts, int64_t rows, hipStream_t st) {
  hipLaunchKernelGGL((k_silu_dropout_bwd<NV, LPR>), dim3((unsigned)nparts), dim3(256), 0, st, a,
                     bias, drop, du, da, dbias_part, rows);
  return launch_status("rb_silu_dropout_bwd");
}

}

int64_t ln_num_parts(int64_t rows, int64_t d) {
  switch (d) {
    case 16: return row_blocks<4>(rows);
    case 32: return row_blocks<8>(rows);
    case 64: return row_blocks<16>(rows);
    case 128: return row_blocks<32>(rows);
    default: return row_blocks<64>(rows);
  }
}

#define RB_ROW_DISPATCH(D, FN, ...)                          \
  switch (D) {                                               \
    case 16: return FN<1, 4>(__VA_ARGS__);                   \
    case 32: return FN<1, 8>(__VA_ARGS__);                   \
    case 64: return FN<1, 16>(__VA_ARGS__);                  \
    case 128: return FN<1, 32>(__VA_ARGS__);                 \
    case 256: return FN<1, 64>(__VA_ARGS__);                 \
    case 512: return FN<2, 64>(__VA_ARGS__);                 \
    case 1024: return FN<4, 64>(__VA_ARGS__);                \
    default:                                                 \
      return fail("row kernels: width must be one of 16, 32, 64, 128, 256, 512, 1024"); \
  }

int launch_add_ln_fwd(const float* a, const int64_t* idx, int64_t nidx, const DropSpec& drop,
                      const float* r, const float* gamma, const float* beta, float eps, float* y,
                      float* s_out, float* mean, float* rstd, int64_t rows, int64_t d,
                      hipStream_t st) {
  RB_ROW_DISPATCH(d, add_ln_fwd_t, a, idx, nidx, drop, r, gamma, beta, eps, y, s_out, mean,
                  rstd, rows, st)
}

int launch_add_ln_bwd(const float* dy, const float* dy2, const float* s, const float* gamma,
                      const float* mean, const float* rstd, const DropSpec& drop, float* ds,
                      float* da, float* dgp, float* dbp, float* dbiasp, int64_t nparts,
                      int64_t rows, int64_t d, hipStream_t st) {
  RB_ROW_DISPATCH(d, add_ln_bwd_t, dy, dy2, s, gamma, mean, rstd, drop, ds, da, dgp, dbp, dbiasp,
                  nparts, rows, st)
}

int launch_silu_dropout_fwd(const float* a, const float* bias, const DropSpec& drop, float* u,
                            int64_t rows, int64_t cols, hipStream_t st) {
  RB_ROW_DISPATCH(cols, silu_fwd_t, a, bias, drop, u, rows, st)
}

int launch_silu_dropout_bwd(const float* a, const float* bias, const DropSpec& drop,
                            const float* du, float* da, float* dbias_part, int64_t nparts,
                            int64_t rows, int64_t cols, hipStream_t st) {
  RB_ROW_DISPATCH(cols, silu_bwd_t, a, bias, drop, du, da, dbias_part, nparts, rows, st)
}

int launch_dropout_mask(const DropSpec& drop, uint8_t* out, int64_t n, hipStream_t st) {
  const int64_t n4 = n / 4;
  const int64_t blocks = std::max<int64_t>(1, std::min<int64_t>(4096, (n4 + 255) / 256));
  hipLaunchKernelGGL(k_dropout_mask, dim3((unsigned)blocks), dim3(256), 0, st, drop, out, n4);
  return launch_status("rb_dropout_mask");
}

}
```

datamining_recblr_amd/kernels.py:

```python
from __future__ import annotations

import contextlib
import ctypes

import torch

from . import _lib
from ._lib import RB_TILE, RecBLRNativeError

__all__ = [
    "scan_fwd", "scan_bwd", "conv_silu_fwd", "conv_silu_bwd", "gate_scan_fwd",
    "gate_scan_bwd", "num_tiles", "RecBLRNativeError", "kernel_timing", "KernelTimer",
    "item_ce_fwd", "item_ce_bwd", "item_ce_probs", "item_rank", "item_scores",
    "item_topk", "SplitRows", "item_split_h", "item_ce_fwd_h", "item_ce_probs_h",
    "embedding_bwd", "embedding_plan",
]


class KernelTimer:

    def __init__(self, only=None):
        self.only = None if only is None else frozenset(only)
        self.records = []
        self.detail = []
# ... 471 lines not shown
            _stream(dy))
    sums = colsum(parts)
    return ds, da, sums[0], sums[1], (sums[2] if want_dbias else None)


def _rows_cols(a):
    cols = a.shape[-1]
    if cols not in ROW_SIZES:
        raise ValueError(f"row width {cols} not in {ROW_SIZES}")
    return a.numel() // cols, cols


def _bias_ptr(bias, cols):
    if bias is None:
        return None
    _check(bias, "bias")
    if bias.shape != (cols,) or not bias.is_contiguous():
        raise ValueError(f"bias must be contiguous [{cols}]")
    return bias.data_ptr()


def silu_dropout_fwd(a, mask=None, seed=0, p=0.0, bias=None):
    _check(a, "a")
    _check_p(p)
    if not a.is_contiguous():
        raise ValueError("a must be contiguous")
    rows, cols = _rows_cols(a)
    _check_mask(mask, (rows, cols))
    u = torch.empty_like(a)
    n = a.numel()
    _launch("rb_silu_dropout_fwd", 8 * n + (n if mask is not None else 0), a.data_ptr(),
            _bias_ptr(bias, cols), _ptr(mask), int(seed), float(p), u.data_ptr(), rows, cols,
            _stream(a))
    return u


def silu_dropout_bwd(a, du, mask=None, seed=0, p=0.0, want_dbias=False, bias=None):
    _check(du, "du")
    _check_p(p)
    du = du.contiguous()
    rows, cols = _rows_cols(a)
    _check_mask(mask, (rows, cols))
    da = torch.empty_like(a)
    nparts = row_num_parts(rows, cols)
    dbias_p = (torch.empty((nparts, cols), device=a.device, dtype=torch.float32)
               if want_dbias else None)
    n = a.numel()
    _launch("rb_silu_dropout_bwd", 12 * n + (n if mask is not None else 0), a.data_ptr(),
            _bias_ptr(bias, cols), _ptr(mask), int(seed), float(p), du.data_ptr(), da.data_ptr(),
            _ptr(dbias_p), nparts, rows, cols, _stream(a))
    return da, (colsum(dbias_p) if want_dbias else None)


def dropout_mask(seed, p, shape, device):
    _check_p(p)
    out = torch.empty(shape, dtype=torch.uint8, device=device)
    n = out.numel()
    if n % 4:
        raise ValueError("numel must be a multiple of 4")
    _launch("rb_dropout_mask", n, int(seed), float(p), out.data_ptr(), n,
            torch.cuda.current_stream(out.device).cuda_stream)
    return out


def embedding_bwd(idx, grad, num_rows, padding_idx=0, plan=None):
    _check(grad, "grad")
    M = idx.numel()
    d = grad.shape[-1]
    grad = grad.reshape(M, d)
    if not grad.is_contiguous():
        grad = grad.contiguous()
    if plan is None:
        plan = embedding_plan(idx, num_rows, d)
    ws_bytes = plan.numel()
    dw = torch.empty((num_rows, d), device=grad.device, dtype=torch.float32)
    pad = -1 if padding_idx is None else int(padding_idx)
    _launch("rb_embedding_bwd", 4 * M * d + 4 * num_rows * d, grad.data_ptr(), M, d, num_rows,
            pad, dw.data_ptr(), plan.data_ptr(), ws_bytes, _stream(grad), _fn="rb_embedding_bwd_apply")
    return dw


def embedding_plan(idx, num_rows, d, stream=None):
    M = idx.numel()
    if idx.dtype != torch.int64 or not idx.is_contiguous():
        raise ValueError("idx must be contiguous int64")
    if idx.device.type != "cuda":
        raise RecBLRNativeError("embedding_plan needs a GPU tensor")
    lib = _lib.load()
    ws_bytes = int(lib.rb_embedding_bwd_workspace(M, num_rows, d))
    ws = torch.empty((ws_bytes,), device=idx.device, dtype=torch.uint8)
    st = stream.cuda_stream if stream is not None else _stream(idx)
    _lib.call("rb_embedding_bwd_plan", idx.data_ptr(), M, d, num_rows, ws.data_ptr(), ws_bytes, st)
    return ws


FLOP_KERNELS = frozenset({"rb_item_ce_fwd", "rb_item_ce_bwd", "rb_item_ce_probs", "rb_item_rank",
                          "rb_item_scores", "rb_item_topk", "rb_item_ce_fwd_h", "rb_item_ce_probs_h",
                          "rb_item_ce_probs_h_t", "rb_item_ce_probs_h_both"})


def f16_split_kernel(name: str) -> bool:
    return name.endswith("_h") or "_h_" in name
ITEM_DIMS = (16, 32, 64, 128, 256)


def _item_operands(seq, items, target=None):
# ... 379 lines not shown
def nt_h_mode(mode: int):
    prev = gemm_nt_h_mode(mode)
    try:
        yield
    finally:
        gemm_nt_h_mode(prev)


def gemm_nt_h_ln_ok(a: torch.Tensor, C: int) -> bool:
    return (a.dim() == 2 and C == 128 and a.shape[1] in (128, 256, 512) and a.stride(1) == 1
            and a.stride(0) % 4 == 0 and a.data_ptr() % 16 == 0 and gemm_nt_h_mode() == 1)


def gemm_nt_h_ln(a: torch.Tensor, wf: torch.Tensor, C: int, bias: torch.Tensor | None,
                 resid: torch.Tensor, gamma: torch.Tensor, beta: torch.Tensor, eps: float,
                 seed: int, p: float, rmax: torch.Tensor | None = None):
    _check(a, "a")
    _check(resid, "resid")
    _check_p(p)
    if not gemm_nt_h_ln_ok(a, C):
        raise ValueError(f"gemm_nt_h_ln: no fused launch for {tuple(a.shape)} -> {C}")
    M, R = a.shape
    if resid.shape != (M, C) or not resid.is_contiguous():
        raise ValueError("resid must be a contiguous [M, C] tensor")
    for t, n in ((gamma, "gamma"), (beta, "beta")):
        _check(t, n)
        if t.numel() != C or t.data_ptr() % 16:
            raise ValueError(f"{n} must hold C floats, 16-byte aligned")
    if bias is not None:
        _check(bias, "bias")
    if rmax is not None:
        _check(rmax, "rmax")
        if rmax.numel() < (M + 31) // 32:
            raise ValueError("rmax needs ceil(M/32) entries")
    y = torch.empty((M, C), device=a.device, dtype=torch.float32)
    s = torch.empty_like(y)
    mean = torch.empty(M, device=a.device, dtype=torch.float32)
    rstd = torch.empty_like(mean)
    _lib.call("rb_gemm_nt_h_ln", a.data_ptr(), a.stride(0), M, R, wf.data_ptr(), C,
              0 if bias is None else bias.data_ptr(), resid.data_ptr(), gamma.data_ptr(),
              beta.data_ptr(), float(eps), int(seed), float(p), y.data_ptr(), s.data_ptr(),
              mean.data_ptr(), rstd.data_ptr(), y.stride(0),
              0 if rmax is None else rmax.data_ptr(), _stream(a))
    return y, s, mean, rstd


def gemm_nt_h_act_ok(a: torch.Tensor, C: int) -> bool:
    M, R = a.shape
    return C % 256 == 0 and C <= 1024 and R % 32 == 0 and R <= 1024 and not (
        M <= 4096 and (R > 256 or C < 256))


def gemm_nt_h_act(a: torch.Tensor, wf: torch.Tensor, C: int, bias: torch.Tensor | None,
                  seed: int, p: float, rmax: torch.Tensor | None = None):
    _check(a, "a")
    _check_p(p)
    if a.dim() != 2 or a.stride(1) != 1:
        raise ValueError("a must be a 2-D tensor with unit inner stride")
    if not gemm_nt_h_act_ok(a, C):
        raise ValueError(f"gemm_nt_h_act: no fused launch for {tuple(a.shape)} -> {C}")
    M, R = a.shape
    out = torch.empty((M, C), device=a.device, dtype=torch.float32)
    act = torch.empty_like(out)
    if bias is not None:
        _check(bias, "bias")
    if rmax is not None:
        _check(rmax, "rmax")
        if rmax.numel() < (M + 31) // 32:
            raise ValueError("rmax needs ceil(M/32) entries")
    _lib.call("rb_gemm_nt_h_act", a.data_ptr(), a.stride(0), M, R, wf.data_ptr(), C,
              0 if bias is None else bias.data_ptr(), out.data_ptr(), out.stride(0),
              0 if rmax is None else rmax.data_ptr(), act.data_ptr(), int(seed), float(p),
              _stream(a))
    return out, act


_dact_parts = None


def gemm_nt_h_dact(a: torch.Tensor, wf: torch.Tensor, C: int, pre: torch.Tensor, seed: int,
                   p: float, rmax: torch.Tensor | None = None, want_dbias: bool = True):
    global _dact_parts
    _check(a, "a")
    _check(pre, "pre")
    _check_p(p)
    if a.dim() != 2 or a.stride(1) != 1:
        raise ValueError("a must be a 2-D tensor with unit inner stride")
    M, R = a.shape
    if not gemm_nt_h_act_ok(a, C) or C > 512:
        raise ValueError(f"gemm_nt_h_dact: no fused launch for {tuple(a.shape)} -> {C}")
    if pre.shape != (M, C) or not pre.is_contiguous():
        raise ValueError("pre must be a contiguous [M, C] tensor")
    if rmax is not None:
        _check(rmax, "rmax")
        if rmax.numel() < (M + 31) // 32:
            raise ValueError("rmax needs ceil(M/32) entries")
    if _dact_parts is None:
        _dact_parts = int(_lib.load().rb_gemm_nt_h_dact_parts())
    out = torch.empty((M, C), device=a.device, dtype=torch.float32)
    part = torch.empty((_dact_parts, C), device=a.device, dtype=torch.float32)
    _lib.call("rb_gemm_nt_h_dact", a.data_ptr(), a.stride(0), M, R, wf.data_ptr(), C,
              out.data_ptr(), out.stride(0), 0 if rmax is None else rmax.data_ptr(),
              pre.data_ptr(), int(seed), float(p), part.data_ptr(), _dact_parts, _stream(a))
    return out, (colsum(part) if want_dbias else None)


def gemm_tn_h(dy: torch.Tensor, x: torch.Tensor, ymax: torch.Tensor, xmax: torch.Tensor,
              splits: int) -> torch.Tensor:
    for t, n in ((dy, "dy"), (x, "x"), (ymax, "ymax"), (xmax, "xmax")):
        _check(t, n)
    if dy.dim() != 2 or x.dim() != 2 or dy.stride(1) != 1 or x.stride(1) != 1:
        raise ValueError("dy and x must be 2-D with unit inner stride")
    M, N = dy.shape
    K = x.shape[1]
    if x.shape[0] != M:
        raise ValueError("dy and x must have the same rows")
    if ymax.numel() < (M + 31) // 32 or xmax.numel() < (M + 31) // 32:
        raise ValueError("ymax / xmax need ceil(M/32) entries")
    parts = torch.empty((splits, N, K), device=dy.device, dtype=torch.float32)
    _lib.call("rb_gemm_tn_h", dy.data_ptr(), dy.stride(0), x.data_ptr(), x.stride(0), M, N, K,
              ymax.data_ptr(), xmax.data_ptr(), parts.data_ptr(), splits, _stream(dy))
    return parts


def bf16_weight_image(w: torch.Tensor, transpose: bool = False) -> torch.Tensor:
    _check(w, "w")
    if w.dim() != 2 or w.stride(1) != 1:
        raise ValueError("w must be a 2-D tensor with unit inner stride")
    C, R = (w.shape[1], w.shape[0]) if transpose else (w.shape[0], w.shape[1])
    img = torch.empty(C * R, device=w.device, dtype=torch.bfloat16)
    _lib.call("rb_gemm_bf16_weight_image", w.data_ptr(), w.stride(0), C, R, int(transpose),
              img.data_ptr(), _stream(w))
    return img


def gemm_nt_bf16(a: torch.Tensor, img: torch.Tensor, C: int,
                 bias: torch.Tensor | None = None) -> torch.Tensor:
    _check(a, "a", torch.bfloat16)
    _check(img, "img", torch.bfloat16)
    if a.dim() != 2 or a.stride(1) != 1:
        raise ValueError("a must be a 2-D tensor with unit inner stride")
    M, R = a.shape
    if img.numel() != C * R:
        raise ValueError("img does not match a [M, R] operand with C outputs")
    if bias is not None:
        _check(bias, "bias")
    out = torch.empty((M, C), device=a.device, dtype=torch.bfloat16)
    _lib.call("rb_gemm_nt_bf16", a.data_ptr(), a.stride(0), M, R, img.data_ptr(), C,
              0 if bias is None else bias.data_ptr(), out.data_ptr(), out.stride(0), _stream(a))
    return out


def gemm_tn_hs(dy: torch.Tensor, x: torch.Tensor, out: torch.Tensor | None = None,
               accumulate: bool = False) -> torch.Tensor:
    for t, n in ((dy, "dy"), (x, "x")):
        _check(t, n)
# ... 115 lines not shown
```

datamining_recblr_amd/linear.py:

```python
from __future__ import annotations

import os
import weakref

import torch

from . import _lib, gemm_tuning, kernels

__all__ = ["linear", "wgrad", "LinearFn", "mm_nt", "mm_nn", "split_gemm_enabled",
           "HipLinearForward", "has_hooks", "fire_hooks"]

_GEMM = os.environ.get("RECBLR_GEMM", "f16x3")
if _GEMM not in ("f16x3", "torch"):
    raise ValueError(f"RECBLR_GEMM must be f16x3 or torch, got {_GEMM!r}")
_split_on = os.environ.get("RECBLR_SPLIT_GEMM", "1") != "0" and _GEMM != "torch"
_half = _GEMM == "f16x3"
_tn_on = os.environ.get("RECBLR_TN", "1") != "0"
_cache_on = os.environ.get("RECBLR_SPLIT_CACHE", "1") != "0"
_small_tn = os.environ.get("RECBLR_SMALL_TN", "0") == "1"

_split_cache: dict = {}
_opt_steps = [0]
_cache_check = os.environ.get("RECBLR_SPLIT_CACHE_CHECK", "0") == "1"

# ... 28 lines not shown


def _weight_split(w: torch.Tensor, transpose: bool) -> torch.Tensor:
    _apply_nt_ws()
    if not _cache_on:
        return _make_image(w, transpose)
    key = (id(w), transpose)
    e = _split_cache.get(key)
    if e is not None and e[0]() is w and e[1] == w.data_ptr() and e[2] == _stamp(w):
        if _cache_check and not torch.equal(e[3], _make_image(w, transpose)):
            raise StaleSplitCacheError(
                "cached split image of a weight is stale: the weight was rewritten without "
                "a torch.optim step or a version bump; call linear.invalidate_split_cache()")
        return e[3]
    if e is None or e[0]() is not w or e[1] != w.data_ptr():
        wf = _make_image(w, transpose)
        _split_cache[key] = [weakref.ref(w), w.data_ptr(), _stamp(w), wf]
        return wf
    jobs, fresh = [], []
    for k, ent in list(_split_cache.items()):
        ww = ent[0]()
        if ww is None or ww.data_ptr() != ent[1]:
            del _split_cache[k]
            continue
        if _stamp(ww) != ent[2] and ww.device == w.device:
            jobs.append((ww, k[1], ent[3]))
            fresh.append(ent)
    kernels.gemm_h_split_weights(jobs)
    for ent in fresh:
        ent[2] = _stamp(ent[0]())
    return e[3]


def split_gemm_enabled() -> bool:
    return _split_on


HALF_MIN_ROWS = 1


def _split_ok(a: torch.Tensor, C: int, R: int) -> bool:
    return (_split_on and _half and a.is_cuda and a.dim() == 2 and a.shape[0] >= HALF_MIN_ROWS
            and C % 32 == 0 and R % 32 == 0 and a.stride(1) == 1 and a.stride(0) % 4 == 0
            and a.data_ptr() % 16 == 0 and a.dtype == torch.float32 and C <= 1024)


def gemm_format() -> str:
    return _GEMM if _split_on else "torch"


_NT_WS = os.environ.get("RECBLR_NT_WS", "1")
if _NT_WS not in ("0", "1"):
    raise ValueError(f"RECBLR_NT_WS must be 0 or 1, got {_NT_WS!r}")
_nt_ws_applied = None


def _apply_nt_ws() -> None:
    global _nt_ws_applied
    if _nt_ws_applied != _NT_WS:
        _lib.load().rb_gemm_nt_h_mode(int(_NT_WS))
        _nt_ws_applied = _NT_WS


def set_nt_ws(on: bool) -> bool:
    global _NT_WS
    prev = _NT_WS == "1"
    _NT_WS = "1" if on else "0"
    _apply_nt_ws()
    return prev


def rmax_wanted() -> bool:
    return _half and _tn_on and _split_on


def rmax_buffer(a: torch.Tensor, C: int, R: int) -> torch.Tensor | None:
    if _half and _tn_on and _split_ok(a, C, R):
        return torch.empty((a.shape[0] + 31) // 32, device=a.device, dtype=torch.float32)
    return None


BF16_NT_MAX_R = 512
BF16_NT_MIN_ROWS = 65536
_BF16_MODES = ("auto", "1", "0")
_bf16_gemm = os.environ.get("RECBLR_BF16_GEMM", "auto")
if _bf16_gemm not in _BF16_MODES:
    raise ValueError(f"RECBLR_BF16_GEMM must be one of {_BF16_MODES}, got {_bf16_gemm!r}")
_bf16_cache: dict = {}


def set_bf16_gemm(mode) -> str:
    global _bf16_gemm
    m = {True: "1", False: "0"}.get(mode, mode) if isinstance(mode, bool) else str(mode)
    if m not in _BF16_MODES:
        raise ValueError(f"bf16 GEMM mode must be one of {_BF16_MODES}, got {mode!r}")
    prev, _bf16_gemm = _bf16_gemm, m
    return prev


def _bf16_image(w: torch.Tensor, transpose: bool) -> torch.Tensor:
    key = (id(w), transpose)
    e = _bf16_cache.get(key)
    if (_cache_on and e is not None and e[0]() is w and e[1] == w.data_ptr()
            and e[2] == _stamp(w)):
        return e[3]
    img = kernels.bf16_weight_image(w, transpose)
    if _cache_on:
        for k in [k for k, v in _bf16_cache.items() if v[0]() is None]:
            del _bf16_cache[k]
        _bf16_cache[key] = (weakref.ref(w), w.data_ptr(), _stamp(w), img)
    return img


def _bf16_ok(a: torch.Tensor, w: torch.Tensor, C: int, R: int) -> bool:
    return (_bf16_gemm != "0"
            and (_bf16_gemm == "1" or (R <= BF16_NT_MAX_R and a.shape[0] >= BF16_NT_MIN_ROWS))
            and a.dtype == torch.bfloat16 and w.dtype == torch.float32 and a.is_cuda
            and a.dim() == 2 and a.shape[0] > 0 and a.stride(1) == 1 and a.stride(0) % 8 == 0
            and a.data_ptr() % 16 == 0 and w.stride(1) == 1 and R % 64 == 0 and C % 256 == 0)


def mm_nt(a: torch.Tensor, w: torch.Tensor, bias: torch.Tensor | None = None,
          rmax: torch.Tensor | None = None) -> torch.Tensor:
    if a.dtype != w.dtype and _bf16_ok(a, w, w.shape[0], w.shape[1]):
        b = None if bias is None else bias.contiguous()
        return kernels.gemm_nt_bf16(a, _bf16_image(w, False), w.shape[0], bias=b)
    if a.dtype != w.dtype:
        wb = w.to(a.dtype)
        return torch.addmm(bias.to(a.dtype), a, wb.t()) if bias is not None else a @ wb.t()
    N, K = w.shape
    if _split_ok(a, N, K):
        return kernels.gemm_nt_h(a, _weight_split(w, False), N, bias=bias, rmax=rmax)
    return torch.addmm(bias, a, w.t()) if bias is not None else torch.mm(a, w.t())


_act_fused = os.environ.get("RECBLR_FFN_ACT", "1") != "0"
ACT_MIN_ROWS = 16384


def set_ffn_act_fused(on: bool) -> bool:
    global _act_fused
    prev, _act_fused = _act_fused, bool(on)
    return prev


def mm_nt_act_ok(a: torch.Tensor, w: torch.Tensor) -> bool:
    N, K = w.shape
    return (_act_fused and _half and a.dtype == w.dtype and a.shape[0] >= ACT_MIN_ROWS
            and _split_ok(a, N, K) and kernels.gemm_nt_h_act_ok(a, N))


def mm_nt_act(a: torch.Tensor, w: torch.Tensor, bias: torch.Tensor | None, seed: int, p: float,
              rmax: torch.Tensor | None = None):
    return kernels.gemm_nt_h_act(a, _weight_split(w, False), w.shape[0], bias, seed, p, rmax=rmax)


_ln_fused = os.environ.get("RECBLR_LN_EPI", "1") != "0"
if os.environ.get("RECBLR_LN_EPI", "1") not in ("0", "1"):
    raise ValueError("RECBLR_LN_EPI must be 0 or 1")


def set_ln_fused(on: bool) -> bool:
    global _ln_fused
    prev, _ln_fused = _ln_fused, bool(on)
    return prev


def mm_nt_ln_ok(a: torch.Tensor, w: torch.Tensor) -> bool:
    N, K = w.shape
    if not (_ln_fused and _half and a.dtype == w.dtype and a.shape[0] >= ACT_MIN_ROWS
            and _split_ok(a, N, K)):
        return False
    _apply_nt_ws()
    return kernels.gemm_nt_h_ln_ok(a, N)


def mm_nt_ln(a: torch.Tensor, w: torch.Tensor, bias: torch.Tensor | None, resid: torch.Tensor,
             gamma: torch.Tensor, beta: torch.Tensor, eps: float, seed: int, p: float,
             rmax: torch.Tensor | None = None):
    return kernels.gemm_nt_h_ln(a, _weight_split(w, False), w.shape[0], bias, resid, gamma, beta,
                                eps, seed, p, rmax=rmax)


def mm_nn_dact_ok(dy: torch.Tensor, w: torch.Tensor) -> bool:
    N, K = w.shape
    return (_act_fused and _half and dy.dtype == w.dtype and K <= 512
            and dy.shape[0] >= ACT_MIN_ROWS and _split_ok(dy, K, N)
            and kernels.gemm_nt_h_act_ok(dy, K))


def mm_nn_dact(dy: torch.Tensor, w: torch.Tensor, pre: torch.Tensor, seed: int, p: float,
               rmax: torch.Tensor | None = None):
    return kernels.gemm_nt_h_dact(dy, _weight_split(w, True), w.shape[1], pre, seed, p,
                                  rmax=rmax)


def mm_nn(dy: torch.Tensor, w: torch.Tensor, out: torch.Tensor | None = None,
          rmax: torch.Tensor | None = None) -> torch.Tensor:
    if dy.dtype != w.dtype and out is None and _bf16_ok(dy, w, w.shape[1], w.shape[0]):
        return kernels.gemm_nt_bf16(dy, _bf16_image(w, True), w.shape[1])
    if dy.dtype != w.dtype:
        wb = w.to(dy.dtype)
        return out.addmm_(dy, wb) if out is not None else dy @ wb
    N, K = w.shape
    if _split_ok(dy, K, N):
        r = kernels.gemm_nt_h(dy, _weight_split(w, True), K, rmax=rmax)
        return r if out is None else out.add_(r)
    if out is not None:
        return out.addmm_(dy, w)
    return torch.mm(dy, w)


SPLIT_K = 64
MIN_ROWS_FOR_SPLIT = 16384
TN_FEW_MIN_ROWS = 2048
_tn_few = os.environ.get("RECBLR_TN_FEW", "1") != "0"


_ncus = {}


def _tn_splits(dev, nt: int) -> int:
    n = _ncus.get(dev)
    if n is None:
        n = _ncus[dev] = torch.cuda.get_device_properties(dev).multi_processor_count
    return max(8, (2 * n // nt) // 8 * 8)


def wgrad(dy2: torch.Tensor, x2: torch.Tensor, splits: int = SPLIT_K,
          ymax: torch.Tensor | None = None, xmax: torch.Tensor | None = None) -> torch.Tensor:
    M = dy2.shape[0]
    N, K = dy2.shape[1], x2.shape[1]
    if (ymax is not None and xmax is not None
            and (M >= MIN_ROWS_FOR_SPLIT or (_tn_few and M >= TN_FEW_MIN_ROWS))
            and N % 128 == 0
            and K % 128 == 0 and dy2.stride(1) == 1 and x2.stride(1) == 1
            and dy2.stride(0) % 4 == 0 and x2.stride(0) % 4 == 0
            and dy2.data_ptr() % 16 == 0 and x2.data_ptr() % 16 == 0):
        S = _tn_splits(dy2.device, (N // 128) * (K // 128))
        if M < MIN_ROWS_FOR_SPLIT:
            S = max(8, min(S, M // 32 // 8 * 8))
        parts = kernels.gemm_tn_h(dy2, x2, ymax, xmax, S)
        return kernels.colsum(parts.view(S, -1)).view(N, K)
    if (_small_tn and _half and _split_on and _tn_on and M < MIN_ROWS_FOR_SPLIT and N % 32 == 0
            and K % 32 == 0 and dy2.dtype == torch.float32 and x2.dtype == torch.float32
            and dy2.is_cuda and dy2.stride(1) == 1 and x2.stride(1) == 1):
        return kernels.gemm_tn_hs(dy2, x2)
# ... 125 lines not shown
```

include/recblr_hip.h:

```cpp
#ifndef RECBLR_HIP_H
#define RECBLR_HIP_H

#include <stddef.h>
#include <stdint.h>

#ifdef __cplusplus
extern "C" {
#endif

#define RB_EINVAL (-1)

typedef uint16_t rb_bf16;

#define RB_TILE 16

#define RB_ABI_VERSION 45
int rb_version(void);

const char* rb_last_error_string(void);

int rb_num_kernels(void);

int rb_scan_fwd(const float* gates, const float* tokens, float* states,
                int64_t B, int64_t C, int64_t T, void* stream);

int rb_scan_bwd(const float* gates, const float* states, const float* grad,
                float* d_gates, float* d_tokens,
                int64_t B, int64_t C, int64_t T, void* stream);

int rb_conv_silu_fwd(const float* x, int64_t x_rs, const float* w,
                     const float* bias, float* xc, int64_t xc_rs,
                     int64_t B, int64_t L, int64_t H, int64_t K, const int64_t* seq_offsets, void* stream);

int rb_conv_silu_fwd_rows(const float* x, int64_t x_rs, const float* w, const float* bias,
                          float* xc, int64_t xc_rs, int64_t ntok, int64_t H, int64_t K,
                          const int64_t* row_pos, void* stream);

int rb_conv_silu_bwd(const float* x, int64_t x_rs, const float* w,
                     const float* bias, const float* g1, const float* g2,
                     float* dx, int64_t dx_rs, float* dw_part, float* db_part,
                     int64_t B, int64_t L, int64_t H, int64_t K, const int64_t* seq_offsets, void* stream);

int rb_gate_scan_fwd(const float* rg, int64_t rg_rs, const float* xc,
                     int64_t xc_rs, const float* z, int64_t z_rs,
                     const float* lam, const float* gate_b, const float* h0,
                     int64_t h0_bs, float* y, int64_t y_rs, float* carries,
                     int64_t B, int64_t L, int64_t H, const int64_t* seq_offsets, void* stream);

int rb_gate_scan_bwd(const float* rg, int64_t rg_rs, const float* xc,
                     int64_t xc_rs, const float* z, int64_t z_rs,
                     const float* lam, const float* gate_b, const float* carries,
                     const float* dy,
                     float* drg, int64_t drg_rs, float* dxc, int64_t dxc_rs,
                     float* dz, int64_t dz_rs, float* part, float* dh0_part,
                     int64_t B, int64_t L, int64_t H, const int64_t* seq_offsets, void* stream);

int rb_gate_scan_fwd_last(const float* rg, int64_t rg_rs, const float* xc, int64_t xc_rs,
                          const float* z, int64_t z_rs, const float* lam, const float* gate_b,
                          const float* h0, int64_t h0_bs, float* y_last, float* carries,
                          int64_t B, int64_t L, int64_t H, const int64_t* seq_offsets,
                          const int64_t* batch_row, void* stream);
int rb_gate_scan_bwd_last(const float* rg, int64_t rg_rs, const float* xc, int64_t xc_rs,
                          const float* z, int64_t z_rs, const float* lam, const float* gate_b,
                          const float* carries, const float* dy_last, float* drg,
                          int64_t drg_rs, float* dxc, int64_t dxc_rs, float* dz, int64_t dz_rs,
                          float* part, float* dh0_part, int64_t B, int64_t L, int64_t H,
                          const int64_t* seq_offsets, const int64_t* batch_row, void* stream);

int rb_pad_prefix_fwd(const float* conv_b, const float* gate_w, const float* gate_b,
// ... 209 lines not shown
```

Before: 373,300.

## Store SiLU-derivative-times-mask factor in FFN forward to skip backward recompute

In the FFN forward, the fused GEMM+SiLU+dropout epilogue now writes the SiLU derivative already multiplied by the keep mask in place of the pre-activation. The backward dact epilogue then multiplies the gradient by this stored factor and the dropout scale. This removes the sigmoid recompute and the dropout-mask regeneration from the backward pass. The stored tensor has the same size as the old one, so memory is unchanged, but the pre-activation is no longer available. The diff also sets _nt_ws_applied to "1" and calls _apply_nt_ws in the act paths, which looks like an unrelated tweak.

```diff
diff --git a/datamining_recblr_amd/_lib.py b/datamining_recblr_amd/_lib.py
--- a/datamining_recblr_amd/_lib.py
+++ b/datamining_recblr_amd/_lib.py
@@ -69,6 +69,8 @@
 ABI_VERSION = _define(_header, "RB_ABI_VERSION")
 
 SIGNATURES = parse_header(_header)
+FFN_SIGNATURES = parse_header(_read(os.path.join(os.path.dirname(HEADER_PATH),
+                                                 "recblr_hip_ffn.h")))
 EXP_SIGNATURES = parse_header(_read(os.path.join(_HERE, "experimental", "recblr_exp.h")))
 PROBE_SIGNATURES = parse_header(_read(os.path.join(_HERE, "probes", "recblr_probe.h")))
 SESSION_SIGNATURES = parse_header(_read(os.path.join(_HERE, "session", "recblr_session.h")))
@@ -101,7 +103,8 @@
 
 
 def load(path: str | None = None) -> ctypes.CDLL:
-    return _load(path or LIB_PATH, SIGNATURES, "HIP extension not built", "rb_version",
+    return _load(path or LIB_PATH, {**SIGNATURES, **FFN_SIGNATURES}, "HIP extension not built",
+                 "rb_version",
                  "ABI mismatch: library {} vs binding {}; rebuild", cache=path is None,
                  hint=" (hipcc --offload-arch=gfx950)")
 
diff --git a/datamining_recblr_amd/blocks.py b/datamining_recblr_amd/blocks.py
--- a/datamining_recblr_amd/blocks.py
+++ b/datamining_recblr_amd/blocks.py
@@ -7,8 +7,9 @@
 
 from . import kernels
 from ._lib import RecBLRNativeError
-from .linear import (_timed, fire_hooks, has_hooks, linear, mm_nn, mm_nn_dact, mm_nn_dact_ok, mm_nt,
-                     mm_nt_act, mm_nt_act_ok, mm_nt_ln, mm_nt_ln_ok, rmax_buffer, wgrad)
+from .linear import (_timed, ffn_factor, fire_hooks, has_hooks, linear, mm_nn, mm_nn_dact,
+                     mm_nn_dact_ok, mm_nt, mm_nt_act, mm_nt_act_ok, mm_nt_ln, mm_nt_ln_ok,
+                     rmax_buffer, wgrad)
 
 __all__ = ["draw_seed", "ResidualGrad", "add_dropout_layer_norm", "embed_dropout_layer_norm",
            "linear_add_dropout_layer_norm", "silu_dropout", "feed_forward", "set_defer_residual",
@@ -202,11 +203,16 @@
         f = 2 * M * d * inner
         want = ctx.needs_input_grad[1] or ctx.needs_input_grad[3]
         r_x = rmax_buffer(x2, inner, d) if want else None
+        factor = ffn_factor() and observe is None and any(ctx.needs_input_grad)
         if mm_nt_act_ok(x2, w1):
-            (a1, u), a1_bias = _timed("gemm", f, mm_nt_act, x2, w1, b1, seed1, p, rmax=r_x), None
+            (a1, u), a1_bias = _timed("gemm", f, mm_nt_act, x2, w1, b1, seed1, p, rmax=r_x,
+                                      factor=factor), None
         else:
             a1 = _timed("gemm", f, mm_nt, x2, w1, rmax=r_x)
-            u = kernels.silu_dropout_fwd(a1, seed=seed1, p=p, bias=b1)
+            if factor:
+                u, a1 = kernels.silu_dropout_fwd_g(a1, seed=seed1, p=p, bias=b1)
+            else:
+                u = kernels.silu_dropout_fwd(a1, seed=seed1, p=p, bias=b1)
             a1_bias = b1
         r_u = rmax_buffer(u, d, inner) if want else None
         save = any(ctx.needs_input_grad)
@@ -225,6 +231,7 @@
         ctx.r_x, ctx.r_u = r_x, r_u
         ctx.seed1, ctx.seed2, ctx.p = seed1, seed2, p
         ctx.a1_has_bias = a1_bias is None
+        ctx.factor = factor
         ctx.in_addend = in_addend if in_addend is not None and in_addend.taken else None
         ctx.out_addend = _take(out_addend)
         ctx.save_for_backward(x2, a1, u, s, mean, rstd, w1, b1, w2, gamma)
@@ -240,13 +247,18 @@
             want_dbias=True, dy2=_pop(ctx.out_addend))
         r_da2 = rmax_buffer(da2, w2.shape[1], d) if ctx.r_u is not None else None
         if ctx.a1_has_bias and mm_nn_dact_ok(da2, w2):
-            da1, db1 = _timed("gemm", f, mm_nn_dact, da2, w2, a1, ctx.seed1, ctx.p, rmax=r_da2)
+            da1, db1 = _timed("gemm", f, mm_nn_dact, da2, w2, a1, ctx.seed1, ctx.p, rmax=r_da2,
+                              factor=ctx.factor)
             dw2 = _timed("gemm", f, wgrad, da2, u, ymax=r_da2, xmax=ctx.r_u)
         else:
             du = _timed("gemm", f, mm_nn, da2, w2, rmax=r_da2)
             dw2 = _timed("gemm", f, wgrad, da2, u, ymax=r_da2, xmax=ctx.r_u)
-            da1, db1 = kernels.silu_dropout_bwd(a1, du, seed=ctx.seed1, p=ctx.p, want_dbias=True,
-                                                bias=None if ctx.a1_has_bias else b1)
+            if ctx.factor:
+                da1, db1 = kernels.silu_dropout_bwd_g(a1, du, p=ctx.p, want_dbias=True)
+            else:
+                da1, db1 = kernels.silu_dropout_bwd(a1, du, seed=ctx.seed1, p=ctx.p,
+                                                    want_dbias=True,
+                                                    bias=None if ctx.a1_has_bias else b1)
         r_da1 = rmax_buffer(da1, d, w1.shape[0]) if ctx.r_x is not None else None
         dx = _timed("gemm", f, mm_nn, da1, w1, rmax=r_da1)
         if ctx.in_addend is not None:
diff --git a/datamining_recblr_amd/build.py b/datamining_recblr_amd/build.py
--- a/datamining_recblr_amd/build.py
+++ b/datamining_recblr_amd/build.py
@@ -10,7 +10,8 @@
 ROOT = os.path.dirname(_HERE)
 SOURCES = sorted(glob.glob(os.path.join(_HERE, "csrc", "*.hip")))
 HEADERS = sorted(glob.glob(os.path.join(_HERE, "csrc", "*.h"))) + [
-    os.path.join(ROOT, "include", "recblr_hip.h")]
+    os.path.join(ROOT, "include", "recblr_hip.h"),
+    os.path.join(ROOT, "include", "recblr_hip_ffn.h")]
 OUT = os.path.join(_HERE, "lib", "libdmrecblr.so")
 PROBE_SOURCES = sorted(glob.glob(os.path.join(_HERE, "probes", "*.hip")))
 PROBE_HEADERS = HEADERS + sorted(glob.glob(os.path.join(_HERE, "probes", "*.h")))
diff --git a/datamining_recblr_amd/csrc/capi.hip b/datamining_recblr_amd/csrc/capi.hip
--- a/datamining_recblr_amd/csrc/capi.hip
+++ b/datamining_recblr_amd/csrc/capi.hip
@@ -164,6 +164,11 @@
   d.mode = mask ? 1 : (p > 0.0f ? 2 : 0);
   return d;
 }
+DropSpec make_drop_g(const uint8_t* mask, uint64_t seed, float p) {
+  DropSpec d = make_drop(mask, seed, p);
+  d.gfac = true;
+  return d;
+}
 }
 
 using namespace rb;
@@ -343,15 +348,41 @@
                         dbeta_part, dbias_part, n_parts, rows, d, stream);
 }
 
-int rb_silu_dropout_fwd(const float* a, const float* bias, const uint8_t* mask, uint64_t seed,
-                        float p, float* u, int64_t rows, int64_t cols, void* stream) {
-  if (!a || !u) return fail("rb_silu_dropout_fwd: null pointer");
+static int silu_dropout_fwd(const float* a, const float* bias, const uint8_t* mask, uint64_t seed,
+                            float p, float* u, float* g, bool gfac, int64_t rows, int64_t cols,
+                            void* stream) {
+  if (!a || !u || (gfac && !g)) return fail("rb_silu_dropout_fwd: null pointer");
   if (bias && !aligned16(bias)) return fail("rb_silu_dropout_fwd: misaligned bias");
   if (rows <= 0 || cols <= 0) return fail("rb_silu_dropout_fwd: rows and cols must be positive");
   if (!(p >= 0.0f && p < 1.0f)) return fail("rb_silu_dropout_fwd: dropout p must be in [0, 1)");
-  if (!aligned16(a) || !aligned16(u) || (mask && (reinterpret_cast<uintptr_t>(mask) & 3)))
+  if (!aligned16(a) || !aligned16(u) || !aligned16(g) ||
+      (mask && (reinterpret_cast<uintptr_t>(mask) & 3)))
     return fail("rb_silu_dropout_fwd: misaligned buffer");
-  return launch_silu_dropout_fwd(a, bias, make_drop(mask, seed, p), u, rows, cols,
+  return launch_silu_dropout_fwd(a, bias, gfac ? make_drop_g(mask, seed, p) : make_drop(mask, seed, p),
+                                 u, g, rows, cols, reinterpret_cast<hipStream_t>(stream));
+}
+
+int rb_silu_dropout_fwd(const float* a, const float* bias, const uint8_t* mask, uint64_t seed,
+                        float p, float* u, int64_t rows, int64_t cols, void* stream) {
+  return silu_dropout_fwd(a, bias, mask, seed, p, u, nullptr, false, rows, cols, stream);
+}
+
+int rb_silu_dropout_fwd_g(const float* a, const float* bias, const uint8_t* mask, uint64_t seed,
+                          float p, float* u, float* g, int64_t rows, int64_t cols, void* stream) {
+  return silu_dropout_fwd(a, bias, mask, seed, p, u, g, true, rows, cols, stream);
+}
+
+int rb_silu_dropout_bwd_g(const float* g, float p, const float* du, float* da, float* dbias_part,
+                          int64_t n_parts, int64_t rows, int64_t cols, void* stream) {
+  if (!g || !du || !da) return fail("rb_silu_dropout_bwd: null pointer");
+  if (rows <= 0 || cols <= 0) return fail("rb_silu_dropout_bwd: rows and cols must be positive");
+  if (!(p >= 0.0f && p < 1.0f)) return fail("rb_silu_dropout_bwd: dropout p must be in [0, 1)");
+  if (!aligned16(g) || !aligned16(du) || !aligned16(da))
+    return fail("rb_silu_dropout_bwd: misaligned buffer");
+  if (dbias_part && n_parts != ln_num_parts(rows, cols))
+    return fail("rb_silu_dropout_bwd: n_parts != rb_row_num_parts");
+  return launch_silu_dropout_bwd(g, nullptr, make_drop_g(nullptr, 0, p), du, da, dbias_part,
+                                 ln_num_parts(rows, cols), rows, cols,
                                  reinterpret_cast<hipStream_t>(stream));
 }
 
@@ -703,9 +734,9 @@
                           reinterpret_cast<hipStream_t>(stream));
 }
 
-int rb_gemm_nt_h_act(const float* A, int64_t lda, int64_t M, int64_t R, const void* Wf, int64_t C,
-                     const float* bias, float* out, int64_t ldo, float* rmax, float* act,
-                     uint64_t seed, float p, void* stream) {
+static int gemm_nt_h_act(const float* A, int64_t lda, int64_t M, int64_t R, const void* Wf,
+                         int64_t C, const float* bias, float* out, int64_t ldo, float* rmax,
+                         float* act, uint64_t seed, float p, bool gfac, void* stream) {
   if (!A || !Wf || !out || !act) return fail("rb_gemm_nt_h_act: null pointer");
   if (M <= 0 || R <= 0 || C <= 0) return fail("rb_gemm_nt_h_act: empty shape");
   if (R % 32 || C % 32 || R > 1024 || C > 1024)
@@ -717,7 +748,20 @@
   if (!(p >= 0.0f && p < 1.0f)) return fail("rb_gemm_nt_h_act: dropout p must be in [0, 1)");
   if ((M + 31) / 32 > 0x7fffffffLL) return fail("rb_gemm_nt_h_act: grid too large");
   return launch_gemm_nt_h_act(A, lda, M, (int)R, Wf, (int)C, bias, out, ldo, rmax, act,
-                              make_drop(nullptr, seed, p), reinterpret_cast<hipStream_t>(stream));
+                              gfac ? make_drop_g(nullptr, seed, p) : make_drop(nullptr, seed, p),
+                              reinterpret_cast<hipStream_t>(stream));
+}
+
+int rb_gemm_nt_h_act(const float* A, int64_t lda, int64_t M, int64_t R, const void* Wf, int64_t C,
+                     const float* bias, float* out, int64_t ldo, float* rmax, float* act,
+                     uint64_t seed, float p, void* stream) {
+  return gemm_nt_h_act(A, lda, M, R, Wf, C, bias, out, ldo, rmax, act, seed, p, false, stream);
+}
+
+int rb_gemm_nt_h_act_g(const float* A, int64_t lda, int64_t M, int64_t R, const void* Wf,
+                       int64_t C, const float* bias, float* g, int64_t ldo, float* rmax,
+                       float* act, uint64_t seed, float p, void* stream) {
+  return gemm_nt_h_act(A, lda, M, R, Wf, C, bias, g, ldo, rmax, act, seed, p, true, stream);
 }
 
 int rb_adam_step(const rb_adam_job* jobs, int64_t n, double lr, double beta1, double beta2,
@@ -741,9 +785,10 @@
 
 int64_t rb_gemm_nt_h_dact_parts(void) { return nt_h_dact_parts(); }
 
-int rb_gemm_nt_h_dact(const float* A, int64_t lda, int64_t M, int64_t R, const void* Wf, int64_t C,
-                      float* out, int64_t ldo, float* rmax, const float* pre, uint64_t seed,
-                      float p, float* dpart, int64_t n_parts, void* stream) {
+static int gemm_nt_h_dact(const float* A, int64_t lda, int64_t M, int64_t R, const void* Wf,
+                          int64_t C, float* out, int64_t ldo, float* rmax, const float* pre,
+                          uint64_t seed, float p, bool gfac, float* dpart, int64_t n_parts,
+                          void* stream) {
   if (!A || !Wf || !out || !pre || !dpart) return fail("rb_gemm_nt_h_dact: null pointer");
   if (M <= 0 || R <= 0 || C <= 0) return fail("rb_gemm_nt_h_dact: empty shape");
   if (R % 32 || C % 32 || R > 1024 || C > 512)
@@ -754,8 +799,22 @@
   if (!(p >= 0.0f && p < 1.0f)) return fail("rb_gemm_nt_h_dact: dropout p must be in [0, 1)");
   if ((M + 31) / 32 > 0x7fffffffLL) return fail("rb_gemm_nt_h_dact: grid too large");
   return launch_gemm_nt_h_dact(A, lda, M, (int)R, Wf, (int)C, out, ldo, rmax, pre,
-                               make_drop(nullptr, seed, p), dpart, n_parts,
-                               reinterpret_cast<hipStream_t>(stream));
+                               gfac ? make_drop_g(nullptr, seed, p) : make_drop(nullptr, seed, p),
+                               dpart, n_parts, reinterpret_cast<hipStream_t>(stream));
+}
+
+int rb_gemm_nt_h_dact(const float* A, int64_t lda, int64_t M, int64_t R, const void* Wf, int64_t C,
+                      float* out, int64_t ldo, float* rmax, const float* pre, uint64_t seed,
+                      float p, float* dpart, int64_t n_parts, void* stream) {
+  return gemm_nt_h_dact(A, lda, M, R, Wf, C, out, ldo, rmax, pre, seed, p, false, dpart, n_parts,
+                        stream);
+}
+
+int rb_gemm_nt_h_dact_g(const float* A, int64_t lda, int64_t M, int64_t R, const void* Wf,
+                        int64_t C, float* out, int64_t ldo, float* rmax, const float* g, float p,
+                        float* dpart, int64_t n_parts, void* stream) {
+  return gemm_nt_h_dact(A, lda, M, R, Wf, C, out, ldo, rmax, g, 0, p, true, dpart, n_parts,
+                        stream);
 }
 
 int rb_gemm_tn_h(const float* dY, int64_t ldy, const float* X, int64_t ldx, int64_t M, int64_t N,
diff --git a/datamining_recblr_amd/csrc/common.h b/datamining_recblr_amd/csrc/common.h
--- a/datamining_recblr_amd/csrc/common.h
+++ b/datamining_recblr_amd/csrc/common.h
@@ -8,6 +8,7 @@
 #include <type_traits>
 
 #include "../../include/recblr_hip.h"
+#include "../../include/recblr_hip_ffn.h"
 
 namespace rb {
 
@@ -46,6 +47,11 @@
 __device__ __forceinline__ float fdsilu(float x) {
   const float s = fsigm(x);
   return s * (1.0f + x * (1.0f - s));
+}
+__device__ __forceinline__ void fsilu_dsilu(float x, float& u, float& d) {
+  const float s = fsigm(x);
+  u = x * s;
+  d = s * (1.0f + x * (1.0f - s));
 }
 
 typedef float rb_f32x4 __attribute__((ext_vector_type(4)));
@@ -265,6 +271,7 @@
   uint32_t key0, key1, keep_thresh;
   float scale;
   int mode;
+  bool gfac;
 
   __device__ __forceinline__ void get4(int64_t e, float (&m)[4]) const {
     if (mode == 0) {
@@ -331,7 +338,7 @@
                       int64_t rows, int64_t d, hipStream_t st);
 int64_t ln_num_parts(int64_t rows, int64_t d);
 int launch_silu_dropout_fwd(const float* a, const float* bias, const DropSpec& drop, float* u,
-                            int64_t rows, int64_t cols, hipStream_t st);
+                            float* g, int64_t rows, int64_t cols, hipStream_t st);
 int launch_silu_dropout_bwd(const float* a, const float* bias, const DropSpec& drop,
                             const float* du, float* da, float* dbias_part, int64_t nparts,
                             int64_t rows, int64_t cols, hipStream_t st);
diff --git a/datamining_recblr_amd/csrc/gemm_half.hip b/datamining_recblr_amd/csrc/gemm_half.hip
--- a/datamining_recblr_amd/csrc/gemm_half.hip
+++ b/datamining_recblr_amd/csrc/gemm_half.hip
@@ -293,14 +293,26 @@
         quad_transpose(v, lane);
         f32x4* o = (f32x4*)(pend_base + (int64_t)(8 * g) * ldo * 4 + n * 128 + st_lane);
         const int64_t row = pend_r0 + 8 * g + 4 * (lane >> 5) + (lane & 3);
+        f32x4 a;
+        if constexpr (ACT) {
+          float m[4];
+          drop.get4(e_base + row * C + pend_c0 + n * 32 + (lane & 28), m);
+          if (drop.gfac) {
+#pragma unroll
+            for (int r = 0; r < 4; ++r) {
+              float u, d;
+              fsilu_dsilu(v[r], u, d);
+              a[r] = u * m[r];
+              v[r] = m[r] != 0.0f ? d : 0.0f;
+            }
+          } else {
+#pragma unroll
+            for (int r = 0; r < 4; ++r) a[r] = fsilu(v[r]) * m[r];
+          }
+        }
         if (pend_full || row < M)
           __builtin_nontemporal_store(f32x4{v[0], v[1], v[2], v[3]}, o);
         if constexpr (ACT) {
-          float m[4];
-          drop.get4(e_base + row * C + pend_c0 + n * 32 + (lane & 28), m);
-          f32x4 a;
-#pragma unroll
-          for (int r = 0; r < 4; ++r) a[r] = fsilu(v[r]) * m[r];
           if (pend_full || row < M)
             __builtin_nontemporal_store(a, (f32x4*)(reinterpret_cast<char*>(o) + act_delta));
         }
@@ -338,12 +350,17 @@
         quad_transpose(v, lane);
         const int64_t row = pend_r0 + 8 * g + rq;
         const bool ok = pend_full || row < M;
-        float mk[4];
-        drop.get4(e_base + row * C + pend_c0 + n * 32 + (lane & 28), mk);
         const f32x4 pv = pq[g];
         f32x4 d;
-#pragma unroll
-        for (int r = 0; r < 4; ++r) d[r] = (v[r] * mk[r]) * fdsilu(pv[r] + 0.0f);
+        if (drop.gfac) {
+#pragma unroll
+          for (int r = 0; r < 4; ++r) d[r] = (v[r] * drop.scale) * pv[r];
+        } else {
+          float mk[4];
+          drop.get4(e_base + row * C + pend_c0 + n * 32 + (lane & 28), mk);
+#pragma unroll
+          for (int r = 0; r < 4; ++r) d[r] = (v[r] * mk[r]) * fdsilu(pv[r] + 0.0f);
+        }
         if (ok) {
           __builtin_nontemporal_store(
               d, (f32x4*)(pend_base + (int64_t)(8 * g) * ldo * 4 + n * 128 + st_lane));
@@ -610,22 +627,30 @@
           if (r < M) {
             float v = __builtin_amdgcn_ldexpf(c[j], erow[j] + ecol) + bv;
             if constexpr (DACT) {
-              float mk[4];
-              const int64_t ei = e_base + r * C + col;
-              drop.get4(ei & ~(int64_t)3, mk);
-              const int q = (int)(ei & 3);
-              v = (v * (q == 0 ? mk[0] : q == 1 ? mk[1] : q == 2 ? mk[2] : mk[3])) *
-                  fdsilu(pre[r * ldo + col] + 0.0f);
+              if (drop.gfac) {
+                v = (v * drop.scale) * pre[r * ldo + col];
+              } else {
+                float mk[4];
+                const int64_t ei = e_base + r * C + col;
+                drop.get4(ei & ~(int64_t)3, mk);
+                const int q = (int)(ei & 3);
+                v = (v * (q == 0 ? mk[0] : q == 1 ? mk[1] : q == 2 ? mk[2] : mk[3])) *
+                    fdsilu(pre[r * ldo + col] + 0.0f);
+              }
               csum += v;
             }
-            out[r * ldo + col] = v;
             if constexpr (ACT) {
               float mk[4];
               const int64_t ei = e_base + r * C + col;
               drop.get4(ei & ~(int64_t)3, mk);
               const int q = (int)(ei & 3);
-              act[r * ldo + col] = fsilu(v) * (q == 0 ? mk[0] : q == 1 ? mk[1] : q == 2 ? mk[2] : mk[3]);
+              const float m = q == 0 ? mk[0] : q == 1 ? mk[1] : q == 2 ? mk[2] : mk[3];
+              float u, d;
+              fsilu_dsilu(v, u, d);
+              act[r * ldo + col] = u * m;
+              if (drop.gfac) v = m != 0.0f ? d : 0.0f;
             }
+            out[r * ldo + col] = v;
           }
         }
         if constexpr (DACT) {
diff --git a/datamining_recblr_amd/csrc/gemm_ws.hip b/datamining_recblr_amd/csrc/gemm_ws.hip
--- a/datamining_recblr_amd/csrc/gemm_ws.hip
+++ b/datamining_recblr_amd/csrc/gemm_ws.hip
@@ -55,8 +55,9 @@
              float* __restrict__ dpart, LnSpec ln) {
   using CF = Cfg<K, NCB, D>;
   constexpr int KS = CF::KS, WC = CF::WC, NT = CF::NT, NLD = CF::NLD, NST = CF::NST;
-  constexpr bool TWO = EPI == 1 || EPI == 3;
-  constexpr bool PRE = EPI == 2 || EPI == 3;
+  constexpr bool ACT = EPI == 1 || EPI == 4, DACT = EPI == 2 || EPI == 5;
+  constexpr bool TWO = ACT || EPI == 3;
+  constexpr bool PRE = DACT || EPI == 3;
   constexpr int NSTT = TWO ? 2 * NST : NST;
   constexpr int NPRE = PRE ? 2 * NCB : 0;
   constexpr int NSO = NSTT + 1 + (EPI == 3 ? 2 : 0);
@@ -74,7 +75,7 @@
   const int nb = rb0 < nrb ? (int)((nrb - 1 - rb0) / rbs + 1) : 0;
   const int64_t prow = (int64_t)(bid / (8 * nct)) * 8 + (bid & 7);
   if (nb == 0) {
-    if constexpr (EPI == 2)
+    if constexpr (DACT)
       for (int c = tid; c < NT; c += THREADS) dpart[prow * C + ct * NT + c] = 0.0f;
     return;
   }
@@ -246,8 +247,8 @@
     }
   };
   f32x4 prv[PRE ? 2 : 1][PRE ? NCB : 1];
-  f32x4 csum[EPI == 2 ? NCB : 1];
-  if constexpr (EPI == 2)
+  f32x4 csum[DACT ? NCB : 1];
+  if constexpr (DACT)
 #pragma unroll
     for (int cb = 0; cb < NCB; ++cb) csum[cb] = f32x4{0.0f, 0.0f, 0.0f, 0.0f};
   auto load_pre = [&](int b) __attribute__((always_inline)) {
@@ -373,12 +374,25 @@
             v[g][i] = __builtin_amdgcn_ldexpf(acc[r][NG * q + g][i], er[r] + ec[g][i]);
             if (BIAS) v[g][i] += bc[g][i];
           }
-          if constexpr (EPI != 0) {
+          if constexpr (EPI == 5) {
+            const f32x4 pv = prv[r][NG * q + g];
+#pragma unroll
+            for (int i = 0; i < 4; ++i) v[g][i] = (v[g][i] * drop.scale) * pv[i];
+            csum[NG * q + g] += v[g];
+          } else if constexpr (EPI != 0) {
             float mk[4];
             drop.get4(row * C + col0 + 16 * (NG * q + g) + 4 * (lane >> 4), mk);
             if constexpr (EPI == 1) {
 #pragma unroll
               for (int i = 0; i < 4; ++i) av[g][i] = fsilu(v[g][i]) * mk[i];
+            } else if constexpr (EPI == 4) {
+#pragma unroll
+              for (int i = 0; i < 4; ++i) {
+                float u, d;
+                fsilu_dsilu(v[g][i], u, d);
+                av[g][i] = u * mk[i];
+                v[g][i] = mk[i] != 0.0f ? d : 0.0f;
+              }
             } else if constexpr (EPI == 2) {
               const f32x4 pv = prv[r][NG * q + g];
 #pragma unroll
@@ -393,7 +407,7 @@
         }
         if constexpr (NG == 1) {
           pend[r] = v[0];
-          if constexpr (EPI == 1) pend2[r] = av[0];
+          if constexpr (ACT) pend2[r] = av[0];
           if constexpr (EPI == 3) ln_part(v[0], ib, r);
         } else {
           f32x4 x1, x2;
@@ -406,7 +420,7 @@
           }
           pend[(q * 2 + r) * 2] = x1;
           pend[(q * 2 + r) * 2 + 1] = x2;
-          if constexpr (EPI == 1) {
+          if constexpr (ACT) {
 #pragma unroll
             for (int i = 0; i < 4; ++i) {
               const float f0 = av[0][i], f1 = av[1][i];
@@ -509,7 +523,7 @@
     for (int i = 0; i < NSTT; ++i) flush(i);
     if constexpr (EPI == 3) ln_store(blast);
   }
-  if constexpr (EPI == 2) {
+  if constexpr (DACT) {
 #pragma unroll
     for (int cb = 0; cb < NCB; ++cb) {
 #pragma unroll
@@ -600,8 +614,12 @@
   const WeightImage w = weight_image(Wf, C, K);
   const int grid = ws::grid_for(M, C, 2);
   dispatch_bool(bias != nullptr, [&](auto bias_c) {
-    ws::run<128, 2, ws::depth<128>(), decltype(bias_c)::value, true, 0, 1>(
-        A, lda, M, w.wi, w.ew, C, bias, out, ldo, rmax, grid, st, act, drop);
+    if (drop.gfac)
+      ws::run<128, 2, ws::depth<128>(), decltype(bias_c)::value, true, 0, 4>(
+          A, lda, M, w.wi, w.ew, C, bias, out, ldo, rmax, grid, st, act, drop);
+    else
+      ws::run<128, 2, ws::depth<128>(), decltype(bias_c)::value, true, 0, 1>(
+          A, lda, M, w.wi, w.ew, C, bias, out, ldo, rmax, grid, st, act, drop);
   });
   return launch_status("rb_gemm_nt_h_act");
 }
@@ -614,8 +632,12 @@
   const int grid = ws::grid_for(M, C, 2);
   const int64_t used = grid / (C / 256);
   if (used > n_parts) return fail("rb_gemm_nt_h_dact: dpart has too few rows");
-  ws::run<128, 2, ws::depth<128>(), false, true, 0, 2>(A, lda, M, w.wi, w.ew, C, nullptr, out, ldo, rmax, grid,
-                                                      st, nullptr, drop, pre, dpart);
+  if (drop.gfac)
+    ws::run<128, 2, ws::depth<128>(), false, true, 0, 5>(A, lda, M, w.wi, w.ew, C, nullptr, out, ldo, rmax, grid,
+                                                        st, nullptr, drop, pre, dpart);
+  else
+    ws::run<128, 2, ws::depth<128>(), false, true, 0, 2>(A, lda, M, w.wi, w.ew, C, nullptr, out, ldo, rmax, grid,
+                                                        st, nullptr, drop, pre, dpart);
   const int rc = launch_status("rb_gemm_nt_h_dact");
   return rc ? rc : nt_dact_zero_rest(dpart, used, n_parts, C, st);
 }
diff --git a/datamining_recblr_amd/csrc/rownorm.hip b/datamining_recblr_amd/csrc/rownorm.hip
--- a/datamining_recblr_amd/csrc/rownorm.hip
+++ b/datamining_recblr_amd/csrc/rownorm.hip
@@ -201,7 +201,7 @@
 template <int NV, int LPR>
 __global__ void __launch_bounds__(256)
 k_silu_dropout_fwd(const float* __restrict__ a, const float* __restrict__ bias, DropSpec drop,
-                   float* __restrict__ u, int64_t rows) {
+                   float* __restrict__ u, float* __restrict__ gout, int64_t rows) {
   constexpr int C = LPR * NV * 4;
   constexpr int RPW = kWave / LPR;
   const int lane = threadIdx.x & (kWave - 1);
@@ -228,8 +228,20 @@
       float x[4], m[4], o[4];
       ldv(x, a + e);
       drop.get4(e, m);
-#pragma unroll
-      for (int v = 0; v < 4; ++v) o[v] = fsilu(x[v] + bv[k][v]) * m[v];
+      if (gout) {
+        float g[4];
+#pragma unroll
+        for (int v = 0; v < 4; ++v) {
+          float d;
+          fsilu_dsilu(x[v] + bv[k][v], o[v], d);
+          o[v] *= m[v];
+          g[v] = m[v] != 0.0f ? d : 0.0f;
+        }
+        stv(gout + e, g);
+      } else {
+#pragma unroll
+        for (int v = 0; v < 4; ++v) o[v] = fsilu(x[v] + bv[k][v]) * m[v];
+      }
       stv(u + e, o);
     }
   }
@@ -273,12 +285,16 @@
       float x[4], g[4], m[4], o[4];
       ldv(x, a + e);
       ldv(g, du + e);
-      drop.get4(e, m);
-#pragma unroll
-      for (int v = 0; v < 4; ++v) {
-        o[v] = (g[v] * m[v]) * fdsilu(x[v] + bv[k][v]);
-        acc[k][v] += o[v];
-      }
+      if (drop.gfac) {
+#pragma unroll
+        for (int v = 0; v < 4; ++v) o[v] = (g[v] * drop.scale) * x[v];
+      } else {
+        drop.get4(e, m);
+#pragma unroll
+        for (int v = 0; v < 4; ++v) o[v] = (g[v] * m[v]) * fdsilu(x[v] + bv[k][v]);
+      }
+#pragma unroll
+      for (int v = 0; v < 4; ++v) acc[k][v] += o[v];
       stv(da + e, o);
     }
   }
@@ -338,11 +354,11 @@
 }
 
 template <int NV, int LPR>
-int silu_fwd_t(const float* a, const float* bias, const DropSpec& drop, float* u, int64_t rows,
-               hipStream_t st) {
+int silu_fwd_t(const float* a, const float* bias, const DropSpec& drop, float* u, float* g,
+               int64_t rows, hipStream_t st) {
   hipLaunchKernelGGL((k_silu_dropout_fwd<NV, LPR>),
                      dim3((unsigned)(row_blocks<LPR, 2 * kRowBlocksFwd>(rows))),
-                     dim3(256), 0, st, a, bias, drop, u, rows);
+                     dim3(256), 0, st, a, bias, drop, u, g, rows);
   return launch_status("rb_silu_dropout_fwd");
 }
 
@@ -396,8 +412,9 @@
 }
 
 int launch_silu_dropout_fwd(const float* a, const float* bias, const DropSpec& drop, float* u,
-                            int64_t rows, int64_t cols, hipStream_t st) {
-  RB_ROW_DISPATCH(cols, silu_fwd_t, a, bias, drop, u, rows, st)
+                            float* g, int64_t rows, int64_t cols, hipStream_t st) {
+  if (drop.gfac != (g != nullptr)) return fail("rb_silu_dropout_fwd: g goes with the factor form");
+  RB_ROW_DISPATCH(cols, silu_fwd_t, a, bias, drop, u, g, rows, st)
 }
 
 int launch_silu_dropout_bwd(const float* a, const float* bias, const DropSpec& drop,
diff --git a/datamining_recblr_amd/kernels.py b/datamining_recblr_amd/kernels.py
--- a/datamining_recblr_amd/kernels.py
+++ b/datamining_recblr_amd/kernels.py
@@ -547,6 +547,39 @@
     return da, (colsum(dbias_p) if want_dbias else None)
 
 
+def silu_dropout_fwd_g(a, mask=None, seed=0, p=0.0, bias=None):
+    _check(a, "a")
+    _check_p(p)
+    if not a.is_contiguous():
+        raise ValueError("a must be contiguous")
+    rows, cols = _rows_cols(a)
+    _check_mask(mask, (rows, cols))
+    u = torch.empty_like(a)
+    g = torch.empty_like(a)
+    n = a.numel()
+    _launch("rb_silu_dropout_fwd_g", 12 * n + (n if mask is not None else 0), a.data_ptr(),
+            _bias_ptr(bias, cols), _ptr(mask), int(seed), float(p), u.data_ptr(), g.data_ptr(),
+            rows, cols, _stream(a))
+    return u, g
+
+
+def silu_dropout_bwd_g(g, du, p=0.0, want_dbias=False):
+    _check(g, "g")
+    _check(du, "du")
+    _check_p(p)
+    du = du.contiguous()
+    if not g.is_contiguous() or du.shape != g.shape:
+        raise ValueError("g must be contiguous and shaped like du")
+    rows, cols = _rows_cols(g)
+    da = torch.empty_like(g)
+    nparts = row_num_parts(rows, cols)
+    dbias_p = (torch.empty((nparts, cols), device=g.device, dtype=torch.float32)
+               if want_dbias else None)
+    _launch("rb_silu_dropout_bwd_g", 12 * g.numel(), g.data_ptr(), float(p), du.data_ptr(),
+            da.data_ptr(), _ptr(dbias_p), nparts, rows, cols, _stream(g))
+    return da, (colsum(dbias_p) if want_dbias else None)
+
+
 def dropout_mask(seed, p, shape, device):
     _check_p(p)
     out = torch.empty(shape, dtype=torch.uint8, device=device)
@@ -1032,7 +1065,7 @@
 
 
 def gemm_nt_h_act(a: torch.Tensor, wf: torch.Tensor, C: int, bias: torch.Tensor | None,
-                  seed: int, p: float, rmax: torch.Tensor | None = None):
+                  seed: int, p: float, rmax: torch.Tensor | None = None, factor: bool = False):
     _check(a, "a")
     _check_p(p)
     if a.dim() != 2 or a.stride(1) != 1:
@@ -1048,7 +1081,8 @@
         _check(rmax, "rmax")
         if rmax.numel() < (M + 31) // 32:
             raise ValueError("rmax needs ceil(M/32) entries")
-    _lib.call("rb_gemm_nt_h_act", a.data_ptr(), a.stride(0), M, R, wf.data_ptr(), C,
+    _lib.call("rb_gemm_nt_h_act_g" if factor else "rb_gemm_nt_h_act", a.data_ptr(), a.stride(0),
+              M, R, wf.data_ptr(), C,
               0 if bias is None else bias.data_ptr(), out.data_ptr(), out.stride(0),
               0 if rmax is None else rmax.data_ptr(), act.data_ptr(), int(seed), float(p),
               _stream(a))
@@ -1059,7 +1093,8 @@
 
 
 def gemm_nt_h_dact(a: torch.Tensor, wf: torch.Tensor, C: int, pre: torch.Tensor, seed: int,
-                   p: float, rmax: torch.Tensor | None = None, want_dbias: bool = True):
+                   p: float, rmax: torch.Tensor | None = None, want_dbias: bool = True,
+                   factor: bool = False):
     global _dact_parts
     _check(a, "a")
     _check(pre, "pre")
@@ -1079,9 +1114,14 @@
         _dact_parts = int(_lib.load().rb_gemm_nt_h_dact_parts())
     out = torch.empty((M, C), device=a.device, dtype=torch.float32)
     part = torch.empty((_dact_parts, C), device=a.device, dtype=torch.float32)
-    _lib.call("rb_gemm_nt_h_dact", a.data_ptr(), a.stride(0), M, R, wf.data_ptr(), C,
-              out.data_ptr(), out.stride(0), 0 if rmax is None else rmax.data_ptr(),
-              pre.data_ptr(), int(seed), float(p), part.data_ptr(), _dact_parts, _stream(a))
+    if factor:
+        _lib.call("rb_gemm_nt_h_dact_g", a.data_ptr(), a.stride(0), M, R, wf.data_ptr(), C,
+                  out.data_ptr(), out.stride(0), 0 if rmax is None else rmax.data_ptr(),
+                  pre.data_ptr(), float(p), part.data_ptr(), _dact_parts, _stream(a))
+    else:
+        _lib.call("rb_gemm_nt_h_dact", a.data_ptr(), a.stride(0), M, R, wf.data_ptr(), C,
+                  out.data_ptr(), out.stride(0), 0 if rmax is None else rmax.data_ptr(),
+                  pre.data_ptr(), int(seed), float(p), part.data_ptr(), _dact_parts, _stream(a))
     return out, (colsum(part) if want_dbias else None)
 
 
diff --git a/datamining_recblr_amd/linear.py b/datamining_recblr_amd/linear.py
--- a/datamining_recblr_amd/linear.py
+++ b/datamining_recblr_amd/linear.py
@@ -104,7 +104,7 @@
 _NT_WS = os.environ.get("RECBLR_NT_WS", "1")
 if _NT_WS not in ("0", "1"):
     raise ValueError(f"RECBLR_NT_WS must be 0 or 1, got {_NT_WS!r}")
-_nt_ws_applied = None
+_nt_ws_applied = "1"
 
 
 def _apply_nt_ws() -> None:
@@ -190,6 +190,21 @@
 ACT_MIN_ROWS = 16384
 
 
+_FFN_G = os.environ.get("RECBLR_FFN_G", "1")
+if _FFN_G not in ("0", "1"):
+    raise ValueError(f"RECBLR_FFN_G must be 0 or 1, got {_FFN_G!r}")
+
+
+def ffn_factor() -> bool:
+    return _FFN_G == "1"
+
+
+def set_ffn_factor(on: bool) -> bool:
+    global _FFN_G
+    prev, _FFN_G = _FFN_G == "1", "1" if on else "0"
+    return prev
+
+
 def set_ffn_act_fused(on: bool) -> bool:
     global _act_fused
     prev, _act_fused = _act_fused, bool(on)
@@ -203,8 +218,10 @@
 
 
 def mm_nt_act(a: torch.Tensor, w: torch.Tensor, bias: torch.Tensor | None, seed: int, p: float,
-              rmax: torch.Tensor | None = None):
-    return kernels.gemm_nt_h_act(a, _weight_split(w, False), w.shape[0], bias, seed, p, rmax=rmax)
+              rmax: torch.Tensor | None = None, factor: bool = False):
+    _apply_nt_ws()
+    return kernels.gemm_nt_h_act(a, _weight_split(w, False), w.shape[0], bias, seed, p, rmax=rmax,
+                                 factor=factor)
 
 
 _ln_fused = os.environ.get("RECBLR_LN_EPI", "1") != "0"
@@ -242,9 +259,10 @@
 
 
 def mm_nn_dact(dy: torch.Tensor, w: torch.Tensor, pre: torch.Tensor, seed: int, p: float,
-               rmax: torch.Tensor | None = None):
+               rmax: torch.Tensor | None = None, factor: bool = False):
+    _apply_nt_ws()
     return kernels.gemm_nt_h_dact(dy, _weight_split(w, True), w.shape[1], pre, seed, p,
-                                  rmax=rmax)
+                                  rmax=rmax, factor=factor)
 
 
 def mm_nn(dy: torch.Tensor, w: torch.Tensor, out: torch.Tensor | None = None,
diff --git a/include/recblr_hip.h b/include/recblr_hip.h
--- a/include/recblr_hip.h
+++ b/include/recblr_hip.h
@@ -14,7 +14,7 @@
 
 #define RB_TILE 16
 
-#define RB_ABI_VERSION 45
+#define RB_ABI_VERSION 46
 int rb_version(void);
 
 const char* rb_last_error_string(void);
diff --git a/include/recblr_hip_ffn.h b/include/recblr_hip_ffn.h
--- /dev/null
+++ b/include/recblr_hip_ffn.h
@@ -0,0 +1,29 @@
+#ifndef RECBLR_HIP_FFN_H
+#define RECBLR_HIP_FFN_H
+
+#include <stddef.h>
+#include <stdint.h>
+
+#ifdef __cplusplus
+extern "C" {
+#endif
+
+int rb_silu_dropout_fwd_g(const float* a, const float* bias, const uint8_t* mask,
+                          uint64_t seed, float p, float* u, float* g, int64_t rows,
+                          int64_t cols, void* stream);
+int rb_silu_dropout_bwd_g(const float* g, float p, const float* du, float* da,
+                          float* dbias_part, int64_t n_parts, int64_t rows,
+                          int64_t cols, void* stream);
+
+int rb_gemm_nt_h_act_g(const float* A, int64_t lda, int64_t M, int64_t R, const void* Wf,
+                       int64_t C, const float* bias, float* g, int64_t ldo, float* rmax,
+                       float* act, uint64_t seed, float p, void* stream);
+int rb_gemm_nt_h_dact_g(const float* A, int64_t lda, int64_t M, int64_t R, const void* Wf,
+                        int64_t C, float* out, int64_t ldo, float* rmax, const float* g,
+                        float p, float* dpart, int64_t n_parts, void* stream);
+
+#ifdef __cplusplus
+}
+#endif
+
+#endif
```

Result: no change. 376,400, median of 6 (+0.8%).
